# mikeoliphant/NeuralAudio

Measured on AMD Instinct MI355X. Metric: concurrent 48 kHz real-time streams + Msamples/s/GPU, NAM WaveNet Standard, higher is better.
Workload: dtype f32 (f16x3-split MFMA, f32 accumulate)

## Files before the change

include/neuralaudio_amd.h:

```cpp
#ifndef NEURALAUDIO_AMD_H
#define NEURALAUDIO_AMD_H

#include "NeuralAudioCApi.h"

#ifdef __cplusplus
extern "C" {
#endif

typedef struct NA_Batch NA_Batch;

NA_EXTERN const char* NA_GetLastError(void);
NA_EXTERN int NA_GetDeviceCount(void);
NA_EXTERN const char* NA_GetVersion(void);

NA_EXTERN NeuralModel* NA_CreateModelFromFileUtf8(NeuralModelLoader* loader, const char* utf8Path, int doPrewarm);
NA_EXTERN NeuralModel* NA_CreateModelFromString(NeuralModelLoader* loader, const char* jsonText, const char* extension, int doPrewarm);
NA_EXTERN void NA_SetDevice(NeuralModelLoader* loader, int device);
NA_EXTERN void NA_SetWaveNetMathMode(NeuralModelLoader* loader, int mathMode);
NA_EXTERN void NA_SetLSTMMathMode(NeuralModelLoader* loader, int mathMode);
NA_EXTERN void NA_SetCompositeModelLoadMode(NeuralModelLoader* loader, int loadMode);
NA_EXTERN int NA_IsQualityChangeRealtimeSafe(NeuralModel* model, float newQuality);
NA_EXTERN int NA_ProcessChecked(NeuralModel* model, float* input, float* output, size_t numSamples);
NA_EXTERN void NA_SetDefaultQualityScaleFactor(NeuralModelLoader* loader, float quality);
NA_EXTERN void NA_SetExternalSampleRate(NeuralModelLoader* loader, int sampleRate);
// ... 73 lines not shown
NA_EXTERN unsigned long long NA_ModelSnapshotFingerprint(NeuralModel* model);
NA_EXTERN int NA_BatchSaveStreams(NA_Batch* batch, const int* streams, int count, void* buf, size_t capacity, size_t* written);
NA_EXTERN int NA_BatchLoadStreams(NA_Batch* batch, const int* streams, int count, const void* buf, size_t bytes);
NA_EXTERN int NA_SaveModelState(NeuralModel* model, void* buf, size_t capacity, size_t* written);
NA_EXTERN int NA_LoadModelState(NeuralModel* model, const void* buf, size_t bytes);

typedef struct NA_MultiBatch NA_MultiBatch;
NA_EXTERN NA_MultiBatch* NA_MultiCreate(const int* devices, int numDevices);
NA_EXTERN void NA_MultiDestroy(NA_MultiBatch* multi);
NA_EXTERN int NA_MultiAddStreams(NA_MultiBatch* multi, NeuralModel* model, float quality, int count, int doPrewarm);
NA_EXTERN int NA_MultiCommit(NA_MultiBatch* multi);
NA_EXTERN int NA_MultiNumStreams(NA_MultiBatch* multi);
NA_EXTERN int NA_MultiNumShards(NA_MultiBatch* multi);
NA_EXTERN int NA_MultiShardRange(NA_MultiBatch* multi, int shard, int* begin, int* end, int* device);
NA_EXTERN int NA_MultiProcess(NA_MultiBatch* multi, const float* in, float* out, size_t n);
NA_EXTERN int NA_MultiSubmit(NA_MultiBatch* multi, const float* in, size_t n);
NA_EXTERN int NA_MultiCollect(NA_MultiBatch* multi, int ticket, float* out);
NA_EXTERN int NA_MultiSetQuality(NA_MultiBatch* multi, int stream, float quality);
NA_EXTERN int NA_MultiSetFanIn(NA_MultiBatch* multi, int mode);
NA_EXTERN const float* NA_MultiGatheredOutput(NA_MultiBatch* multi, int shard);
NA_EXTERN int NA_RcclAvailable(void);
NA_EXTERN int NA_ShardByCost(const double* cost, int n, int parts, int* bounds);
NA_EXTERN double NA_ModelStreamCost(NeuralModel* model, float quality);

NA_EXTERN int NA_ModelKernelInfo(NeuralModel* model, float quality, int streams, char* kernelBuf, int bufSize, float* inputLimit, int* rangeProven,
	int* weightsOk, int* packFactor);

NA_EXTERN float NA_BatchStreamInputLimit(NA_Batch* batch, int stream);
NA_EXTERN int NA_BatchStreamRangeEvents(NA_Batch* batch, int stream);

typedef struct NA_RenderJob
{
	NeuralModel* model;
	float quality;
	const float* input;
	float* output;
	size_t numSamples;
} NA_RenderJob;
typedef struct NA_RenderOptions
{
	size_t segmentSamples;
	size_t maxSamplesPerPass;
	double waitLimitMs;
} NA_RenderOptions;
typedef struct NA_RenderPlanInfo
{
	long long segments;
	int lead;
	long long segmentSamples;
	long long rowSamples;
	int passes;
	int streams;
	double estimatedMs;
	char kernel[64];
} NA_RenderPlanInfo;
NA_EXTERN int NA_RenderOffline(const NA_RenderJob* jobs, int numJobs, const NA_RenderOptions* opts);
NA_EXTERN int NA_RenderPlan(const NA_RenderJob* jobs, int numJobs, const NA_RenderOptions* opts, NA_RenderPlanInfo* info);

typedef struct NA_ResampleInfo {
	int externalRate, modelRate;
	int ticksExternal, ticksModel;
	int tapsUp, tapsDown;
	int quantum;
	int latencySamples;
	int prototypeLength;
} NA_ResampleInfo;
NA_EXTERN int NA_ResamplePlan(int externalRate, int modelRate, int quantum, NA_ResampleInfo* info);
NA_EXTERN int NA_ResamplePrototype(int externalRate, int modelRate, float* buf, int capacity);
NA_EXTERN long long NA_ResampleModelFrames(int externalRate, int modelRate, int quantum, long long externalSamples);
NA_EXTERN int NA_BatchSetResampling(NA_Batch* batch, int externalRate, int modelRate, int quantum, int maxFrames);
NA_EXTERN int NA_BatchGetResampleInfo(NA_Batch* batch, NA_ResampleInfo* info);
NA_EXTERN void NA_SetResampleToExternalRate(NeuralModelLoader* loader, int on);
NA_EXTERN int NA_GetProcessLatencySamples(NeuralModel* model);
NA_EXTERN int NA_GetModelProcessRate(NeuralModel* model);
NA_EXTERN int NA_RenderOfflineAtRate(const NA_RenderJob* jobs, int numJobs, const NA_RenderOptions* opts, int externalRate);
NA_EXTERN int NA_RenderPlanAtRate(const NA_RenderJob* jobs, int numJobs, const NA_RenderOptions* opts, int externalRate,
                                  NA_RenderPlanInfo* info, NA_ResampleInfo* resample);
NA_EXTERN int NA_MultiSetResampling(NA_MultiBatch* multi, int externalRate, int modelRate, int quantum, int maxFrames);
NA_EXTERN int NA_MultiGetResampleInfo(NA_MultiBatch* multi, NA_ResampleInfo* info);
#ifndef NA_RELEASE
NA_EXTERN int NA_DebugClassifyNam(const char* jsonText);
NA_EXTERN int NA_DebugPackedWeights(NeuralModel* model, int* packFactor, float* out, int capacity);
NA_EXTERN int NA_DebugSplitPlan(NeuralModel* model, int* stages, int stageCapacity, unsigned short* wsplit, long long wsplitCapacity, long long* wsplitCount);
NA_EXTERN void NA_DebugSetWaveNetSpec(int on);
NA_EXTERN int NA_DebugSetRecurrentQuadMin(int streams);
NA_EXTERN long long NA_DebugRecurrentQuadLaunches(void);
NA_EXTERN int NA_DebugRecurrentPlan(NeuralModel* model, int out[6]);
NA_EXTERN int NA_DebugRecurrentShapePlan(int cell, int hidden, int numLayers, int tailLayers, int tailWidth, int tailHistory, int rpl, int forceL2w, int out[6]);
NA_EXTERN int NA_DebugRecurrentKernel(int cell, int hidden, int numLayers, int tailLayers, int tailWidth, int tailHistory, int haveWT, int knobMask, int rpl,
	char* outName, int cap);
NA_EXTERN long long NA_DebugSnapshotLaunches(void);
NA_EXTERN void NA_DebugSetRcclApi(int mode, int failSendAt, int rendezvousMs);
NA_EXTERN int NA_DebugStallDevice(NA_Batch* batch, double milliseconds);
NA_EXTERN long long NA_DebugDeviceResourceCalls(void);
NA_EXTERN int NA_DebugResampleTap(NA_Batch* batch, float* modelIn, float* modelOut, long long capacityPerRow, int* frames);
NA_EXTERN void NA_DebugSetRenderTap(float* modelIn, float* modelOut, long long capacity);
NA_EXTERN void NA_DebugSetTraceBuffer(void* deviceBuffer);
NA_EXTERN int NA_DebugRunCabinetStage(NA_Batch* batch, float* hostRows, long stride, size_t n);
NA_EXTERN long long NA_DebugCabinetLaunches(void);
NA_EXTERN long long NA_DebugGateLaunches(void);
#endif

#ifdef __cplusplus
}
#endif
#endif
```

neuralaudio_amd/capi.py:

```python
import ctypes as C
import os

_HERE = os.path.dirname(os.path.abspath(__file__))
_SUFFIX = os.environ.get("NA_LIB_SUFFIX", "")
LIB_PATH = (os.path.join(os.path.dirname(_HERE), "tools", "variants", "libNeuralAudioCAPI%s.so" % _SUFFIX) if _SUFFIX
            else os.path.join(_HERE, "libNeuralAudioCAPI.so"))

LEGACY_SYMBOLS = [
    "CreateLoader", "DeleteLoader", "CreateModelFromFile", "DeleteModel", "SetLSTMLoadMode", "SetWaveNetLoadMode",
    "SetAudioInputLevelDBu", "SetDefaultMaxAudioBufferSize", "GetLoadMode", "IsStatic", "SetMaxAudioBufferSize",
    "GetRecommendedInputDBAdjustment", "GetRecommendedOutputDBAdjustment", "GetSampleRate", "Process",
]

NA_SYMBOLS = [
    "NA_GetLastError", "NA_GetDeviceCount", "NA_GetVersion", "NA_CreateModelFromFileUtf8", "NA_CreateModelFromString",
    "NA_SetDevice", "NA_SetDefaultQualityScaleFactor", "NA_SetExternalSampleRate", "NA_HasQualityScaling",
    "NA_GetQualityScaleFactor", "NA_SetQualityScaleFactor", "NA_GetReceptiveFieldSize", "NA_Prewarm", "NA_GetMetadata",
    "NA_GetModelVersion", "NA_BatchCreate", "NA_BatchDestroy", "NA_BatchAddStreams", "NA_BatchNumStreams",
    "NA_BatchSetQuality", "NA_BatchGetActiveSubModel", "NA_BatchPrewarm", "NA_BatchProcess", "NA_BatchProcessDevice",
    "NA_BatchSynchronize", "NA_BatchGetHipStream", "NA_BatchAlgorithmicBytesPerSample", "NA_BatchMacsPerSample",
    "NA_BatchStateBytes", "NA_BatchStreamPackFactor", "NA_BatchStreamKernelName", "NA_DebugSetTraceBuffer", "NA_DebugSetWaveNetSpec", "NA_DebugSetRecurrentQuadMin", "NA_DebugRecurrentQuadLaunches", "NA_RegisterHostBuffer", "NA_UnregisterHostBuffer", "NA_BatchStreamInputLimit", "NA_BatchRemoveStreams", "NA_MultiCreate", "NA_MultiDestroy", "NA_MultiAddStreams", "NA_MultiCommit", "NA_MultiNumStreams", "NA_MultiNumShards", "NA_MultiShardRange", "NA_MultiProcess", "NA_MultiSubmit", "NA_MultiCollect", "NA_MultiSetQuality", "NA_ShardByCost", "NA_ModelStreamCost", "NA_BatchNumLiveStreams", "NA_BatchIsLive", "NA_SetWaveNetMathMode", "NA_SetLSTMMathMode", "NA_SetCompositeModelLoadMode",
    "NA_IsQualityChangeRealtimeSafe", "NA_ProcessChecked", "NA_BatchSubmit", "NA_BatchCollect", "NA_BatchNextInput", "NA_BatchOutputView", "NA_BatchIsQualityChangeRealtimeSafe", "NA_DebugClassifyNam", "NA_DebugPackedWeights", "NA_DebugSplitPlan", "NA_ModelKernelInfo", "NA_BatchStreamRangeEvents", "NA_MultiSetFanIn", "NA_MultiGatheredOutput", "NA_RcclAvailable",
    "NA_BatchMarkTime", "NA_BatchWaitMarks", "NA_BatchElapsedMs", "NA_BatchUsesHalfLaunches", "NA_DebugSetRcclApi", "NA_BatchWaitOutputs", "NA_BatchUsesResidentLaunch", "NA_BatchSetResidentLaunch",
    "NA_BatchSetWaitLimitMs", "NA_BatchGetWaitLimitMs", "NA_BatchIsBroken", "NA_DebugStallDevice",
    "NA_RenderOffline", "NA_RenderPlan",
    "NA_BatchStreamSnapshotBytes", "NA_ModelSnapshotBytes", "NA_ModelSnapshotFingerprint", "NA_BatchSaveStreams", "NA_BatchLoadStreams",
    "NA_SaveModelState", "NA_LoadModelState", "NA_DebugSnapshotLaunches",
    "NA_ResamplePlan", "NA_ResamplePrototype", "NA_ResampleModelFrames", "NA_BatchSetResampling", "NA_BatchGetResampleInfo",
    "NA_SetResampleToExternalRate", "NA_GetProcessLatencySamples", "NA_GetModelProcessRate", "NA_DebugResampleTap",
    "NA_RenderOfflineAtRate", "NA_RenderPlanAtRate", "NA_DebugSetRenderTap", "NA_MultiSetResampling", "NA_MultiGetResampleInfo",
    "NA_BatchReserveStreams", "NA_BatchActivateStream", "NA_BatchParkStream", "NA_BatchIsParked", "NA_BatchFindParked", "NA_BatchNumParked",
    "NA_DebugDeviceResourceCalls", "NA_DebugRecurrentPlan", "NA_DebugRecurrentShapePlan", "NA_DebugRecurrentKernel",
    "NA_BatchEnableOutputStage", "NA_BatchSetStreamGain", "NA_BatchGetStreamGain", "NA_BatchHandover", "NA_BatchHandoverRemaining",
    "NA_BatchEnableCabinetStage", "NA_BatchGetCabinetInfo", "NA_BatchLoadIR", "NA_BatchUnloadIR", "NA_BatchSetStreamIR", "NA_BatchGetStreamIR",
    "NA_BatchStreamIRFadeRemaining", "NA_DebugRunCabinetStage", "NA_DebugCabinetLaunches",
    "NA_GateParamsFromDb", "NA_BatchEnableGateStage", "NA_BatchGetGateInfo", "NA_BatchSetStreamGate", "NA_BatchGetStreamGate",
    "NA_BatchStreamGateGain", "NA_DebugGateLaunches",
]


class NA_RenderJob(C.Structure):
    _fields_ = [("model", C.c_void_p), ("quality", C.c_float), ("input", C.POINTER(C.c_float)), ("output", C.POINTER(C.c_float)),
                ("numSamples", C.c_size_t)]


class NA_RenderOptions(C.Structure):
    _fields_ = [("segmentSamples", C.c_size_t), ("maxSamplesPerPass", C.c_size_t), ("waitLimitMs", C.c_double)]


class NA_RenderPlanInfo(C.Structure):
    _fields_ = [("segments", C.c_longlong), ("lead", C.c_int), ("segmentSamples", C.c_longlong), ("rowSamples", C.c_longlong),
                ("passes", C.c_int), ("streams", C.c_int), ("estimatedMs", C.c_double), ("kernel", C.c_char * 64)]


class NA_ResampleInfo(C.Structure):
    _fields_ = [("externalRate", C.c_int), ("modelRate", C.c_int), ("ticksExternal", C.c_int), ("ticksModel", C.c_int),
                ("tapsUp", C.c_int), ("tapsDown", C.c_int), ("quantum", C.c_int), ("latencySamples", C.c_int),
                ("prototypeLength", C.c_int)]


class NA_CabinetInfo(C.Structure):
    _fields_ = [("maxTaps", C.c_int), ("ringSamples", C.c_int), ("pieceSamples", C.c_int), ("numIRs", C.c_int), ("deviceBytes", C.c_longlong)]


class NA_GateParams(C.Structure):
    _fields_ = [("openPower", C.c_float), ("closePower", C.c_float), ("floorGain", C.c_float), ("detectorCoeff", C.c_float),
                ("attackSamples", C.c_int), ("holdSamples", C.c_int), ("releaseSamples", C.c_int)]


class NA_GateInfo(C.Structure):
    _fields_ = [("gainSamples", C.c_int), ("numGates", C.c_int), ("deviceBytes", C.c_longlong)]


_lib = None


def load_library():
    global _lib
    if _lib is not None:
        return _lib
    if not os.path.exists(LIB_PATH):
        raise OSError("libNeuralAudioCAPI.so not found at %s -- build it with `python -c 'import __graft_entry__ as g; "
                      "g.build()'` (there is no CPU fallback)" % LIB_PATH)
    lib = C.CDLL(LIB_PATH, mode=C.RTLD_GLOBAL)
    fp = C.POINTER(C.c_float)
    vp = C.c_void_p
    sig = {
        "CreateLoader": (vp, []),
        "DeleteLoader": (None, [vp]),
        "CreateModelFromFile": (vp, [vp, C.c_wchar_p]),
        "DeleteModel": (None, [vp]),
        "SetLSTMLoadMode": (None, [vp, C.c_int]),
        "SetWaveNetLoadMode": (None, [vp, C.c_int]),
        "SetAudioInputLevelDBu": (None, [vp, C.c_float]),
        "SetDefaultMaxAudioBufferSize": (None, [vp, C.c_int]),
        "GetLoadMode": (C.c_int, [vp]),
        "IsStatic": (C.c_bool, [vp]),
        "SetMaxAudioBufferSize": (None, [vp, C.c_int]),
        "GetRecommendedInputDBAdjustment": (C.c_float, [vp]),
        "GetRecommendedOutputDBAdjustment": (C.c_float, [vp]),
        "GetSampleRate": (C.c_float, [vp]),
        "Process": (None, [vp, fp, fp, C.c_size_t]),
        "NA_GetLastError": (C.c_char_p, []),
        "NA_GetDeviceCount": (C.c_int, []),
        "NA_GetVersion": (C.c_char_p, []),
# ... 54 lines not shown
        "NA_DebugDeviceResourceCalls": (C.c_longlong, []),
        "NA_BatchEnableOutputStage": (C.c_int, [vp]),
        "NA_BatchSetStreamGain": (C.c_int, [vp, C.c_int, C.c_float, C.c_int]),
        "NA_BatchGetStreamGain": (C.c_float, [vp, C.c_int]),
        "NA_BatchHandover": (C.c_int, [vp, C.c_int, C.c_int, C.c_float, C.c_int]),
        "NA_BatchHandoverRemaining": (C.c_int, [vp, C.c_int]),
        "NA_BatchEnableCabinetStage": (C.c_int, [vp, C.c_int]),
        "NA_BatchGetCabinetInfo": (C.c_int, [vp, C.POINTER(NA_CabinetInfo)]),
        "NA_BatchLoadIR": (C.c_int, [vp, fp, C.c_int]),
        "NA_BatchUnloadIR": (C.c_int, [vp, C.c_int]),
        "NA_BatchSetStreamIR": (C.c_int, [vp, C.c_int, C.c_int, C.c_int]),
        "NA_BatchGetStreamIR": (C.c_int, [vp, C.c_int]),
        "NA_BatchStreamIRFadeRemaining": (C.c_int, [vp, C.c_int]),
        "NA_DebugRunCabinetStage": (C.c_int, [vp, fp, C.c_long, C.c_size_t]),
        "NA_DebugCabinetLaunches": (C.c_longlong, []),
        "NA_GateParamsFromDb": (C.c_int, [C.c_int] + [C.c_float] * 7 + [C.POINTER(NA_GateParams)]),
        "NA_BatchEnableGateStage": (C.c_int, [vp]),
        "NA_BatchGetGateInfo": (C.c_int, [vp, C.POINTER(NA_GateInfo)]),
        "NA_BatchSetStreamGate": (C.c_int, [vp, C.c_int, C.POINTER(NA_GateParams), C.c_int]),
        "NA_BatchGetStreamGate": (C.c_int, [vp, C.c_int, C.POINTER(NA_GateParams)]),
        "NA_BatchStreamGateGain": (C.c_float, [vp, C.c_int]),
        "NA_DebugGateLaunches": (C.c_longlong, []),
        "NA_DebugRecurrentPlan": (C.c_int, [vp, C.POINTER(C.c_int)]),
        "NA_DebugRecurrentShapePlan": (C.c_int, [C.c_int] * 8 + [C.POINTER(C.c_int)]),
        "NA_DebugRecurrentKernel": (C.c_int, [C.c_int] * 9 + [C.c_char_p, C.c_int]),
        "NA_MultiCreate": (vp, [C.POINTER(C.c_int), C.c_int]),
        "NA_MultiDestroy": (None, [vp]),
        "NA_MultiAddStreams": (C.c_int, [vp, vp, C.c_float, C.c_int, C.c_int]),
        "NA_MultiCommit": (C.c_int, [vp]),
        "NA_MultiNumStreams": (C.c_int, [vp]),
        "NA_MultiNumShards": (C.c_int, [vp]),
        "NA_MultiShardRange": (C.c_int, [vp, C.c_int, C.POINTER(C.c_int), C.POINTER(C.c_int), C.POINTER(C.c_int)]),
        "NA_MultiProcess": (C.c_int, [vp, C.POINTER(C.c_float), C.POINTER(C.c_float), C.c_size_t]),
        "NA_MultiSubmit": (C.c_int, [vp, C.POINTER(C.c_float), C.c_size_t]),
        "NA_MultiCollect": (C.c_int, [vp, C.c_int, C.POINTER(C.c_float)]),
        "NA_MultiSetQuality": (C.c_int, [vp, C.c_int, C.c_float]),
        "NA_ShardByCost": (C.c_int, [C.POINTER(C.c_double), C.c_int, C.c_int, C.POINTER(C.c_int)]),
        "NA_ModelStreamCost": (C.c_double, [vp, C.c_float]),
        "NA_BatchStreamRangeEvents": (C.c_int, [vp, C.c_int]),
        "NA_MultiSetFanIn": (C.c_int, [vp, C.c_int]),
        "NA_MultiGatheredOutput": (vp, [vp, C.c_int]),
        "NA_RcclAvailable": (C.c_int, []),
        "NA_ModelKernelInfo": (C.c_int, [vp, C.c_float, C.c_int, C.c_char_p, C.c_int, fp, C.POINTER(C.c_int), C.POINTER(C.c_int), C.POINTER(C.c_int)]),
        "NA_BatchNumLiveStreams": (C.c_int, [vp]),
        "NA_BatchIsLive": (C.c_int, [vp, C.c_int]),
        "NA_SetWaveNetMathMode": (None, [vp, C.c_int]),
        "NA_SetLSTMMathMode": (None, [vp, C.c_int]),
        "NA_SetCompositeModelLoadMode": (None, [vp, C.c_int]),
        "NA_IsQualityChangeRealtimeSafe": (C.c_int, [vp, C.c_float]),
        "NA_ProcessChecked": (C.c_int, [vp, fp, fp, C.c_size_t]),
        "NA_BatchSubmit": (C.c_int, [vp, fp, C.c_size_t]),
        "NA_BatchCollect": (C.c_int, [vp, C.c_int, fp]),
        "NA_BatchNextInput": (fp, [vp, C.c_size_t]),
        "NA_BatchOutputView": (fp, [vp, C.c_int]),
        "NA_BatchIsQualityChangeRealtimeSafe": (C.c_int, [vp, C.c_int, C.c_float]),
        "NA_DebugClassifyNam": (C.c_int, [C.c_char_p]),
        "NA_DebugPackedWeights": (C.c_int, [vp, C.POINTER(C.c_int), C.POINTER(C.c_float), C.c_int]),
        "NA_RenderOffline": (C.c_int, [C.POINTER(NA_RenderJob), C.c_int, C.POINTER(NA_RenderOptions)]),
        "NA_RenderPlan": (C.c_int, [C.POINTER(NA_RenderJob), C.c_int, C.POINTER(NA_RenderOptions), C.POINTER(NA_RenderPlanInfo)]),
        "NA_BatchStreamSnapshotBytes": (C.c_longlong, [vp, C.c_int]),
        "NA_ModelSnapshotBytes": (C.c_longlong, [vp]),
        "NA_ModelSnapshotFingerprint": (C.c_ulonglong, [vp]),
        "NA_BatchSaveStreams": (C.c_int, [vp, C.POINTER(C.c_int), C.c_int, vp, C.c_size_t, C.POINTER(C.c_size_t)]),
        "NA_BatchLoadStreams": (C.c_int, [vp, C.POINTER(C.c_int), C.c_int, vp, C.c_size_t]),
        "NA_SaveModelState": (C.c_int, [vp, vp, C.c_size_t, C.POINTER(C.c_size_t)]),
        "NA_LoadModelState": (C.c_int, [vp, vp, C.c_size_t]),
        "NA_DebugSnapshotLaunches": (C.c_longlong, []),
        "NA_ResamplePlan": (C.c_int, [C.c_int, C.c_int, C.c_int, C.POINTER(NA_ResampleInfo)]),
        "NA_ResamplePrototype": (C.c_int, [C.c_int, C.c_int, fp, C.c_int]),
        "NA_ResampleModelFrames": (C.c_longlong, [C.c_int, C.c_int, C.c_int, C.c_longlong]),
        "NA_BatchSetResampling": (C.c_int, [vp, C.c_int, C.c_int, C.c_int, C.c_int]),
        "NA_BatchGetResampleInfo": (C.c_int, [vp, C.POINTER(NA_ResampleInfo)]),
        "NA_SetResampleToExternalRate": (None, [vp, C.c_int]),
        "NA_GetProcessLatencySamples": (C.c_int, [vp]),
        "NA_GetModelProcessRate": (C.c_int, [vp]),
        "NA_DebugResampleTap": (C.c_int, [vp, fp, fp, C.c_longlong, C.POINTER(C.c_int)]),
        "NA_RenderOfflineAtRate": (C.c_int, [C.POINTER(NA_RenderJob), C.c_int, C.POINTER(NA_RenderOptions), C.c_int]),
        "NA_RenderPlanAtRate": (C.c_int, [C.POINTER(NA_RenderJob), C.c_int, C.POINTER(NA_RenderOptions), C.c_int, C.POINTER(NA_RenderPlanInfo),
                                          C.POINTER(NA_ResampleInfo)]),
        "NA_DebugSetRenderTap": (None, [fp, fp, C.c_longlong]),
        "NA_MultiSetResampling": (C.c_int, [vp, C.c_int, C.c_int, C.c_int, C.c_int]),
        "NA_MultiGetResampleInfo": (C.c_int, [vp, C.POINTER(NA_ResampleInfo)]),
        "NA_DebugSplitPlan": (C.c_int, [vp, C.POINTER(C.c_int), C.c_int, C.POINTER(C.c_ushort), C.c_longlong, C.POINTER(C.c_longlong)]),
    }
    for name, (res, args) in sig.items():
        try:
            fn = getattr(lib, name)
        except AttributeError:
            if os.environ.get("NA_LIB_SUFFIX") and name.startswith("NA_"):
                continue
            raise
        fn.restype = res
        fn.argtypes = args
    _lib = lib
    return lib


def last_error():
    return load_library().NA_GetLastError().decode("utf-8", "replace")


def device_count():
    return int(load_library().NA_GetDeviceCount())
```

neuralaudio_amd/csrc/capi.cpp:

```cpp
#include <cstring>
#include <cwchar>
#include <string>

#include "neuralaudio_amd.h"
#include "multi_gpu.h"
#include "offline_render.h"
#include "resample.h"
#include "stream_snapshot.h"
#include "neural_model_impl.h"
#include "lstm_launch.h"
#include "wavenet_launch.h"
#include "wavenet_plan.h"
#include "tuning.h"

struct NeuralModel
{
	NeuralAudio::NeuralModel* model;
};

struct NeuralModelLoader
{
	NeuralAudio::NeuralModelLoader* loader;
};

// ... 198 lines not shown
}

int NA_ProcessChecked(NeuralModel* model, float* input, float* output, size_t numSamples)
{
	if (!model || !output)
	{
		SetError("Process: null argument");
		return -1;
	}
	const int rc = Guard([&] { model->model->Process(input, output, numSamples); });
	if (rc != 0) memset(output, 0, numSamples * sizeof(float));
	return rc;
}

void NA_SetWaveNetMathMode(NeuralModelLoader* loader, int mathMode)
{
	if (loader) loader->loader->SetWaveNetMathMode(mathMode == 1 ? NeuralAudio::EMathMode::StdMath : NeuralAudio::EMathMode::FastMath);
}

void NA_SetLSTMMathMode(NeuralModelLoader* loader, int mathMode)
{
	if (loader) loader->loader->SetLSTMMathMode(mathMode == 1 ? NeuralAudio::EMathMode::StdMath : NeuralAudio::EMathMode::FastMath);
}

void NA_SetCompositeModelLoadMode(NeuralModelLoader* loader, int loadMode)
{
	if (loader) loader->loader->SetCompositeModelLoadMode(loadMode == 1 ? NeuralAudio::ECompositeModelLoadMode::OnDemand : NeuralAudio::ECompositeModelLoadMode::LoadAll);
}

int NA_IsQualityChangeRealtimeSafe(NeuralModel* model, float newQuality)
{
	return (model && model->model->IsQualityChangeRealtimeSafe(newQuality)) ? 1 : 0;
}

#ifndef NA_RELEASE
int NA_DebugClassifyNam(const char* jsonText)
{
	int r = -1;
	Guard([&] {
		const na::Json j = na::Json::Parse(jsonText ? jsonText : "");
		const std::string v = (j.IsObject() && j.Contains("version") && j.At("version").IsString()) ? j.At("version").AsString() : "";
		r = (na::NAMIsA2(v) ? 1 : 0) | (na::NAMIsA2Standard(j) ? 2 : 0);
	});
	return r;
}
#endif

#ifndef NA_RELEASE
int NA_DebugPackedWeights(NeuralModel* model, int* packFactor, float* out, int capacity)
{
	int r = -1;
	Guard([&] {
		NeuralAudio::GpuModel* gm = model ? dynamic_cast<NeuralAudio::GpuModel*>(model->model) : nullptr;
		if (!gm) throw std::runtime_error("NA_DebugPackedWeights: not a model of this library");
		const auto& lm = gm->GetLoadedModel();
		if (lm->subModels.size() != 1 || lm->subModels[0].desc->kind != na::MODEL_WAVENET)
		{
			if (packFactor) *packFactor = 1;
			r = 0;
			return;
		}
		const na::WaveNetDesc& wn = lm->subModels[0].desc->wavenet;
		const int P = na::WaveNetPackFactor(wn);
		if (packFactor) *packFactor = P;
		if (P < 2)
		{
			r = 0;
			return;
		}
		const bool dense = na::Tuning::Get().wnDense != 0 && na::WaveNetPackCanBeDense(wn, P);
		const na::WaveNetDesc v = na::PackWaveNetDesc(wn, P, dense);
		na::ValidateWaveNetDesc(v);
		const na::WaveNetPlan plan = na::BuildPackedWaveNetPlan(wn, P, dense);
		if (plan.pack != P || plan.splitFastT != 2) throw std::runtime_error("NA_DebugPackedWeights: the packed plan is not a fast split-kernel plan");
		r = (int)v.weights.size();
		if (out)
			for (int i = 0; i < r && i < capacity; i++) out[i] = v.weights[(size_t)i];
	});
	return r;
}
#endif

#ifndef NA_RELEASE
int NA_DebugSplitPlan(NeuralModel* model, int* stages, int stageCapacity, unsigned short* wsplit, long long wsplitCapacity, long long* wsplitCount)
{
	int r = -1;
	Guard([&] {
		NeuralAudio::GpuModel* gm = model ? dynamic_cast<NeuralAudio::GpuModel*>(model->model) : nullptr;
		if (!gm) throw std::runtime_error("NA_DebugSplitPlan: not a model of this library");
		const auto& lm = gm->GetLoadedModel();
		if (lm->subModels.size() != 1 || lm->subModels[0].desc->kind != na::MODEL_WAVENET) throw std::runtime_error("NA_DebugSplitPlan: not a WaveNet");
		const na::WaveNetPlan plan = na::BuildWaveNetPlan(lm->subModels[0].desc->wavenet, true);
		static_assert(sizeof(na::WnSplitStage) == 16 * sizeof(int), "16 ints per stage");
		r = (int)plan.sstages.size();
		if (stages) memcpy(stages, plan.sstages.data(), sizeof(na::WnSplitStage) * (size_t)std::min(r, stageCapacity));
		if (wsplitCount) *wsplitCount = (long long)plan.wsplit.size();
		if (wsplit) memcpy(wsplit, plan.wsplit.data(), sizeof(uint16_t) * (size_t)std::min<long long>((long long)plan.wsplit.size(), wsplitCapacity));
	});
	return r;
}
#endif

#ifndef NA_RELEASE
int NA_DebugRecurrentShapePlan(int cell, int hidden, int numLayers, int tailLayers, int tailWidth, int tailHistory, int rpl, int forceL2w, int out[6])
{
	if (!out || (cell != 0 && cell != 1) || hidden < 1 || numLayers < 0 || tailLayers < 0) return -1;
	const na::RecurrentPlan p = na::RecurrentWavePlan(cell == 1 ? na::LSTM_CELL_GRU : na::LSTM_CELL_LSTM, hidden, numLayers, tailLayers, tailWidth, tailHistory, true, rpl, forceL2w);
	out[0] = p.runs; out[1] = p.waves; out[2] = p.rowsPerLane; out[3] = p.l2w; out[4] = p.headInLoop; out[5] = (int)p.ldsBytes;
	return na::RecurrentWaveShape(hidden, numLayers, tailLayers > 0 ? tailWidth : 0, tailLayers > 0 ? tailHistory : 0) ? 1 : 0;
}
#endif

#ifndef NA_RELEASE
int NA_DebugRecurrentKernel(int cell, int hidden, int numLayers, int tailLayers, int tailWidth, int tailHistory, int haveWT, int knobMask, int rpl, char* outName, int cap)
{
	if ((cell != 0 && cell != 1) || hidden < 1 || numLayers < 0 || tailLayers < 0 || knobMask < -1 || knobMask > 63) return -1;
	const int b = knobMask;
	const na::RecurrentKnobs k = b < 0 ? na::RecurrentKnobs::FromTuning()
		: na::RecurrentKnobs{ (b & 1) != 0, (b & 2) != 0, (b & 4) != 0, (b & 8) != 0, (b & 16) != 0, rpl > 0 ? rpl : 1, (b & 32) != 0 };
	const na::RecurrentKernel kernel = na::RecurrentKernelFor(cell == 1 ? na::LSTM_CELL_GRU : na::LSTM_CELL_LSTM, hidden, numLayers, tailLayers, tailWidth, tailHistory,
		haveWT != 0, k).kernel;
	if (outName && cap > 0) snprintf(outName, (size_t)cap, "%s", na::RecurrentKernelName(kernel));
	return (int)kernel;
}
#endif

#ifndef NA_RELEASE
int NA_DebugRecurrentPlan(NeuralModel* model, int out[6])
{
	int r = -1;
	Guard([&] {
		NeuralAudio::GpuModel* gm = model ? dynamic_cast<NeuralAudio::GpuModel*>(model->model) : nullptr;
		if (!gm || !out) throw std::runtime_error("NA_DebugRecurrentPlan: not a model of this library");
		const auto& lm = gm->GetLoadedModel();
		if (lm->subModels.size() != 1 || lm->subModels[0].desc->kind != na::MODEL_LSTM) throw std::runtime_error("NA_DebugRecurrentPlan: not a recurrent model");
		const na::LSTMDesc& d = lm->subModels[0].desc->lstm;
		int tailWidth = 0, tailHistory = 0;
		na::RecurrentTailDims(d, tailWidth, tailHistory);
		const na::RecurrentPlan p = na::RecurrentWavePlan(d.cell == na::CELL_GRU ? na::LSTM_CELL_GRU : na::LSTM_CELL_LSTM, d.hiddenSize, d.numLayers, (int)d.tail.size(),
			tailWidth, tailHistory);
		out[0] = p.runs; out[1] = p.waves; out[2] = p.rowsPerLane; out[3] = p.l2w; out[4] = p.headInLoop; out[5] = (int)p.ldsBytes;
		r = 0;
	});
	return r;
}
#endif

void NA_SetDevice(NeuralModelLoader* loader, int device)
{
	if (loader) loader->loader->SetDevice(device);
}

void NA_SetDefaultQualityScaleFactor(NeuralModelLoader* loader, float quality)
{
	if (loader) loader->loader->SetDefaultQualityScaleFactor(quality);
}

void NA_SetExternalSampleRate(NeuralModelLoader* loader, int sampleRate)
{
	if (loader) loader->loader->SetExternalSampleRate(sampleRate);
}

int NA_HasQualityScaling(NeuralModel* model) { return (model && model->model->HasQualityScaling()) ? 1 : 0; }

float NA_GetQualityScaleFactor(NeuralModel* model) { return model ? model->model->GetQualityScaleFactor() : 1.0f; }

void NA_SetQualityScaleFactor(NeuralModel* model, float quality)
{
	if (model) Guard([&] { model->model->SetQualityScaleFactor(quality); });
}

int NA_GetReceptiveFieldSize(NeuralModel* model) { return model ? model->model->GetReceptiveFieldSize() : -1; }

int NA_Prewarm(NeuralModel* model)
{
	if (!model) return -1;
	return Guard([&] { model->model->Prewarm(); });
}

int NA_GetMetadata(NeuralModel* model, const char* fieldName, char* buf, int bufSize)
// ... 962 lines not shown
```

neuralaudio_amd/csrc/tuning.cpp:

```cpp
#include "tuning.h"

#include <cstdlib>
#include <cstring>

namespace na
{
	namespace
	{
#ifndef NA_NO_TUNING
		bool Has(const char* name) { return getenv(name) != nullptr; }
		int Int(const char* name, int dflt)
		{
			const char* e = getenv(name);
			return e ? atoi(e) : dflt;
		}
		bool IsZero(const char* name)
		{
			const char* e = getenv(name);
			return e != nullptr && atoi(e) == 0;
		}
#endif
		Tuning Parse()
		{
			Tuning t;
#ifndef NA_NO_TUNING
			if (const char* e = getenv("NA_WN_KERNEL")) t.wnKernel = !strcmp(e, "split") ? 1 : (!strcmp(e, "frame") ? 2 : (!strcmp(e, "generic") ? 3 : 0));
			t.wnPack = Int("NA_WN_PACK", -1);
			t.wnPadOff = IsZero("NA_WN_PAD");
			t.wnNtOff = IsZero("NA_WN_NT");
			t.wnNtFromMB = Int("NA_WN_NT_MB", 400);
			t.wnDense = Int("NA_WN_DENSE", -1);
			t.spT = Int("NA_SP_T", 0);
			t.spSpb = Int("NA_SP_SPB", 0);
			t.spGen = Has("NA_SP_GEN");
			t.wnSpecOff = IsZero("NA_WN_SPEC") || Has("NA_SP_T") || Has("NA_SP_GEN");
			t.spNoT1 = Has("NA_SP_NO_T1");
			t.spReverse = Has("NA_SP_REVERSE");
			t.frPrefetch = Int("NA_FR_PF", 1);
			t.frSpb = Int("NA_FR_SPB", 0);
			t.traceBlock = Int("NA_TRACE_BLOCK", 0);
			t.traceChain = Int("NA_TRACE_CHAIN", 0);
			t.lstmNoDpp = Has("NA_LSTM_NO_DPP");
			t.gruNoDpp = Has("NA_GRU_NO_DPP");
			t.lstmLaneKernel = Has("NA_LSTM_LANE_KERNEL");
			t.lstmNoWaveRt = Has("NA_LSTM_NO_WAVE_RT");
			t.recL2w = Int("NA_REC_L2W", 0) != 0;
			t.recQuadMin = Int("NA_REC_QUAD_MIN", -1);
			t.recNoDpp32 = Has("NA_REC_NO_DPP32");
			t.recNoSkew = Has("NA_REC_NOSKEW");
			t.recNoPipe = Has("NA_REC_NOPIPE");
			t.recPipeMax = Int("NA_REC_PIPE_MAX", 0);
			t.recRpl = Int("NA_REC_RPL", 1);
			t.hostChains = Int("NA_HOST_CHAINS", 2);
			t.hostHalvesOff = IsZero("NA_HOST_HALVES");
			t.hostDirect = !IsZero("NA_HOST_DIRECT");
			t.batchSerial = Has("NA_BATCH_SERIAL");
			t.batchNoGraph = Has("NA_BATCH_NO_GRAPH");
			t.residentOn = Int("NA_RESIDENT", 0) != 0;
			t.residentHostRing = Int("NA_RESIDENT_HOST_RING", 0) != 0;
			t.residentDelayUs = Int("NA_RESIDENT_DELAY_US", 0);
			t.residentGrid = Int("NA_RESIDENT_GRID", 0);
			t.residentIdleUs = Int("NA_RESIDENT_IDLE_US", 200);
#endif
			return t;
		}
	}

	const Tuning& Tuning::Get()
	{
		static const Tuning t = Parse();
		return t;
	}
}
```

neuralaudio_amd/csrc/tuning.h:

```cpp
#pragma once

namespace na
{
	struct Tuning
	{
		int wnKernel = 0;
		int wnPack = -1;
		int wnDense = -1;
		int wnNtFromMB = 400;
		bool wnNtOff = false;
		bool wnPadOff = false;
		bool wnSpecOff = false;
		int spT = 0;
		int spSpb = 0;
		bool spGen = false;
		bool spNoT1 = false;
		bool spReverse = false;
		int frPrefetch = 1;
		int frSpb = 0;
		int traceBlock = 0;
		int traceChain = 0;
		bool lstmNoDpp = false;
		bool gruNoDpp = false;
		bool lstmLaneKernel = false;
		bool lstmNoWaveRt = false;
		bool recL2w = false;
		int recQuadMin = -1;
		bool recNoDpp32 = false;
		bool recNoSkew = false;
		bool recNoPipe = false;
		int recPipeMax = 0;
		int recRpl = 1;
		int hostChains = 2;
		bool hostHalvesOff = false;
		bool hostDirect = true;
		bool batchSerial = false;
		bool batchNoGraph = false;
		bool residentOn = false;
		bool residentHostRing = false;
		int residentDelayUs = 0;
		int residentGrid = 0;
		int residentIdleUs = 200;

		static const Tuning& Get();
	};
}
```

neuralaudio_amd/csrc/wavenet_dev.h:

```cpp
#pragma once

#include <cstdint>

namespace na
{
	constexpr int WN_TILE = 16;
	constexpr int WN_MAX_TILES = 8;
	constexpr int WN_MAX_FRAMES = WN_TILE * WN_MAX_TILES;
	constexpr int WN_MAX_RINGS = 64;
	constexpr int WN_HEADER_F4 = WN_MAX_RINGS / 4;
	constexpr int WN_RANGE_EVENT_SLOT = WN_MAX_RINGS - 1;

	constexpr int WN_COMPACT_MAX_HISTORY = 32;
	constexpr int WnRingKeep(int ringFrames) { return ringFrames < WN_MAX_FRAMES ? ringFrames / 3 : ringFrames - WN_MAX_FRAMES; }
	constexpr bool WnCompactSafeFrames(int n) { return (n >= 1 && n <= 32) || n == 64 || n == 128; }

	enum WnStageType : int
	{
		WN_ST_RECHANNEL_COND = 0,
		WN_ST_LAYER = 1,
		WN_ST_ARRAY_LINK = 2,
		WN_ST_HEAD_DENSE_OUT = 3,
		WN_ST_HEAD_CONV_OUT = 4,
	};

	enum WnStageFlags : int
	{
		WN_FLAG_LEAKY = 1,
		WN_FLAG_NEED_OUTPUT = 2,
		WN_FLAG_PUBLISH = 4,
		WN_FLAG_BIAS = 8,
		WN_FLAG_STD_TANH = 16,
		WN_FLAG_FOLD = 32,
	};

	struct WnStage
	{
		int type;
		int flags;
		int G;
		int ksize;
		int dilation;
		int ring_id;
		int ring_off;
		int ring_frames;
		int out_ring_id;
		int out_ring_off;
		int out_ring_frames;
		int out_G;
		int a4_off;
		int a4_floats;
		int vec_off;
		int pk_conv_off;
		int pk_w1_off;
		int reserved[15];
	};
	static_assert(sizeof(WnStage) == 128, "stage descriptors are 128-byte records");


	struct WnSplitStage
	{
		int type;
		int flags;
		int G;
		int Gp;
		int ksize;
		int dilation;
		int ring_off;
		int ring_frames;
		int ring_id;
		int out_ring_off;
		int out_ring_frames;
		int out_ring_id;
		int out_G;
		int a_off;
		int a_ops;
		int reserved;
	};
	static_assert(sizeof(WnSplitStage) == 64, "split stage descriptors are 64-byte records");

	constexpr int WN_GENERIC_MAX_CHANNELS = 128;
	constexpr int WN_COL_STRIDE = 128;

	struct WnPrewarmLayer
	{
		int kind;
		int cin, cout, ksize;
		int act;
		int wconv;
		int bconv;
		int wmix;
		int w1, b1;
		int ring_id;
		int need_output;
		int last_of_array;
		int rechannel;
		int rech_in;
		int dilation;
	};

	struct WnModelDev
	{
		const WnStage* stages;
		const float* wpack;
		const float* wpk;
		const int* ring_frames;
		int nstages;
		int wpack_f4;
		int max_a4_floats;
		int max_ksize;
		int wpk_floats;
		int nrings;
		int state_f4;
		float head_scale;
		const WnSplitStage* sstages;
		const void* wsplit;
		int wsplit_quads;
		int max_split_ops;
		int max_G;
		int split_fast_T;
		int spec_arch;
		float cond_limit;
		int compact_rings;
		int saturate;
	};

	enum WnSpecArch : int
	{
		WN_SPEC_NONE = 0,
		WN_SPEC_STD = 1,
		WN_SPEC_LITE = 2,
		WN_SPEC_LITE16 = 3,
		WN_SPEC_A2FULL = 4,
		WN_SPEC_A2LITE = 5,
	};
}
```

neuralaudio_amd/csrc/wavenet_launch.h:

```cpp
#pragma once

#include <cstring>
#include <vector>

#include <hip/hip_runtime_api.h>

#include "device_resources.h"
#include "tuning.h"
#include "wavenet_dev.h"

namespace na
{
	constexpr int WN_FRAME_MAX_GROUPS = 8;
	struct WnFrameGroup
	{
		const WnModelDev* model;
		float* state;
		const int* slots;
		const int* rows;
		int numStreams, slot0, row0;
		int pack;
	};
	hipError_t LaunchWaveNetFrameFused(const WnFrameGroup* groups, int numGroups, const float* in, float* out, long inStride, long outStride, int n,
		hipStream_t stream);
// ... 31 lines not shown
			entries.clear();
		}
		void NewGeneration(unsigned long g)
		{
			if (g != generation) Clear();
			generation = g;
		}
		hipError_t Ensure(const void* fresh, size_t bytes, hipStream_t stream, const void** dev)
		{
			for (const Entry& e : entries)
				if (e.host.size() == bytes && memcmp(e.host.data(), fresh, bytes) == 0)
				{
					*dev = e.dev;
					return hipSuccess;
				}
			hipStreamCaptureStatus capturing = hipStreamCaptureStatusNone;
			(void)hipStreamIsCapturing(stream, &capturing);
			if (capturing != hipStreamCaptureStatusNone) return hipErrorStreamCaptureUnsupported;
			if (entries.size() >= 16) Clear();
			Entry e;
			hipError_t err = CountedHipMalloc(&e.dev, bytes);
			if (err != hipSuccess) return err;
			err = hipMemcpy(e.dev, fresh, bytes, hipMemcpyHostToDevice);
			if (err != hipSuccess)
			{
				(void)CountedHipFree(e.dev);
				return err;
			}
			e.host.assign(static_cast<const char*>(fresh), static_cast<const char*>(fresh) + bytes);
			*dev = e.dev;
			entries.push_back(std::move(e));
			return hipSuccess;
		}
	};
	hipError_t LaunchWaveNetSpecTable(const WnFrameGroup* groups, int numGroups, const float* in, float* out, long inStride, long outStride, int n,
		hipStream_t stream, WnLaunchTable& table);

	constexpr int RESIDENT_RING = 64;
	struct ResidentCmd
	{
		const float* in;
		float* out;
		long inStride, outStride;
		unsigned long long seq;
		unsigned long long check;
		unsigned long long pad[2];
	};
#ifdef __HIPCC__
	__host__ __device__
#endif
	inline unsigned long long ResidentCmdCheck(unsigned long long in, unsigned long long out, unsigned long long inStride, unsigned long long outStride, unsigned long long seq)
	{
		return seq * 0x9E3779B97F4A7C15ull + in * 0xC2B2AE3D27D4EB4Full + out * 0x165667B19E3779F9ull + inStride * 0xD6E8FEB86659FD93ull + outStride * 0xFF51AFD7ED558CCDull + 1ull;
	}
	struct ResidentCtrl
	{
		unsigned long long exitAfter;
		unsigned long long pad0[7];
		ResidentCmd cmd[RESIDENT_RING];
	};
	struct ResidentStatus
	{
		unsigned long long completed;
		unsigned long long pad1[7];
	};
	static_assert(sizeof(ResidentCmd) == 64 && sizeof(ResidentCtrl) == 64 + 64 * RESIDENT_RING && sizeof(ResidentStatus) == 64, "command ring layout");
	struct ResidentArgs
	{
		const ResidentCtrl* ctrl;
		ResidentStatus* status;
		unsigned* doneCount;
		unsigned* wgDone;
		unsigned long long base;
		int numBlocks;
		unsigned idleTicks;
		unsigned startDelay;
	};
	hipError_t LaunchWaveNetSpecResident(const WnFrameGroup* groups, int numGroups, int n, const ResidentArgs& ra, hipStream_t stream, int* gridOut);
	int WaveNetSpecResidentGrid(const WnFrameGroup* groups, int numGroups, int n);

	bool WaveNetSpecEnabled();
	void SetWaveNetSpecEnabled(bool on);
	int WaveNetSpecArchId(const WnSplitStage* stages, int nstages, int stateF4, int wsplitQuads);

	hipError_t LaunchWaveNetGeneric(const WnPrewarmLayer* layers, int numLayers, const float* weights, const int* ringOffF4, const int* ringFrames,
		const int* ringG, int nrings, int stateF4, int maxChannels, float headScale, float condLimit, bool saturate, float* state, const int* slots, const int* rows,
		int numStreams, int slot0, int row0, const float* in, float* out, long inStride, long outStride, int n, hipStream_t stream);

	hipError_t LaunchWaveNetFrame(const WnModelDev& m, float* state, const int* slots, const int* rows, int numStreams, const float* in,
		float* out, long inStride, long outStride, int n, hipStream_t stream, int slot0 = 0, int row0 = 0);

	void SetWaveNetTraceBuffer(long long* deviceBuffer);
	long long* GetWaveNetTraceBuffer();

	hipError_t LaunchWaveNetPrewarmColumns(const WnPrewarmLayer* layers, int numLayers, const float* weights, float* cols,
		hipStream_t stream);

	hipError_t LaunchWaveNetFillRings(float* state, int stateF4, const int* slots, int numStreams, int numRings, const int* ringOffF4,
		const int* ringFrames, const int* ringG, const float* cols, hipStream_t stream, bool splitFormat, const int* sub = nullptr, int pack = 1,
		bool zero = false);

	hipError_t LaunchWaveNetRearm(float* state, int stateF4, const int* entries, int numEntries, int numRings, const int* ringOffF4,
		const int* ringFrames, const int* ringG, const float* cols, hipStream_t stream, bool splitFormat, int pack);
}
```

neuralaudio_amd/csrc/wavenet_plan.cpp:

```cpp
#include "wavenet_plan.h"
#include "frame_lds.h"

#include <algorithm>
#include <cmath>
#include <cstring>
#include <functional>
#include <sstream>
#include <stdexcept>

namespace na
{
	static int CeilDiv(int a, int b) { return (a + b - 1) / b; }

	size_t WaveNetDesc::ExpectedNumWeights() const
	{
		size_t n = 0;
		for (const auto& a : arrays)
		{
			const size_t c = (size_t)a.channels;
			n += c * a.inputSize;
			for (size_t l = 0; l < a.kernelSizes.size(); l++)
			{
				n += c * c * a.kernelSizes[l] + c;
				n += c * a.conditionSize;
// ... 19 lines not shown
	{
		if (desc.arrays.empty()) throw std::runtime_error("WaveNet without layer arrays");
		const int numArrays = (int)desc.arrays.size();
		int rings = 0;
		for (int a = 0; a < numArrays; a++)
		{
			const WnArrayCfg& cfg = desc.arrays[a];
			if (cfg.channels < 1 || cfg.headSize < 1 || cfg.inputSize < 1) throw std::runtime_error("WaveNet layer array with a zero-sized dimension");
			if (cfg.channels > WN_GENERIC_MAX_CHANNELS || cfg.headSize > WN_GENERIC_MAX_CHANNELS || cfg.inputSize > WN_GENERIC_MAX_CHANNELS)
				throw std::runtime_error("WaveNet channels > 128 are not supported");
			if (cfg.headKernelSize > 1 && (cfg.channels > 64 || cfg.headSize > 64))
				throw std::runtime_error("WaveNet: a conv head on a layer array wider than 64 channels is not supported");
			if (cfg.conditionSize != 1) throw std::runtime_error("WaveNet condition_size != 1 is not supported");
			if (cfg.kernelSizes.size() != cfg.dilations.size() || cfg.kernelSizes.empty())
				throw std::runtime_error("WaveNet kernel_sizes/dilations mismatch");
			for (size_t l = 0; l < cfg.kernelSizes.size(); l++)
				if (cfg.kernelSizes[l] < 1 || cfg.dilations[l] < 1) throw std::runtime_error("WaveNet kernel_size / dilation must be >= 1");
			if (cfg.headKernelSize < 1 || cfg.headDilation < 1) throw std::runtime_error("WaveNet head kernel_size / dilation must be >= 1");
			rings += (int)cfg.kernelSizes.size() + (cfg.headKernelSize > 1 ? 1 : 0);
			if (a > 0)
			{
				if (desc.arrays[a - 1].headSize != cfg.channels || cfg.inputSize != desc.arrays[a - 1].channels)
					throw std::runtime_error("WaveNet layer arrays do not chain (head_size/input_size mismatch)");
				if (desc.arrays[a - 1].headKernelSize != 1)
					throw std::runtime_error("WaveNet: head kernel > 1 is only supported on the last layer array");
			}
		}
		if (desc.arrays[0].inputSize != 1) throw std::runtime_error("WaveNet first layer array must have input_size 1");
		if (rings > WN_MAX_RINGS) throw std::runtime_error("WaveNet has more than 64 conv layers (unsupported)");
		const size_t expected = desc.ExpectedNumWeights();
		if (expected != desc.weights.size())
		{
			std::stringstream str;
			str << "Wrong number of weights. Expected " << expected << " but got " << desc.weights.size();
			throw std::runtime_error(str.str());
		}
	}


	static uint16_t FloatToHalfBits(float f)
	{
		uint32_t x;
		memcpy(&x, &f, 4);
		const uint32_t sign = (x >> 16) & 0x8000u;
		x &= 0x7fffffffu;
		if (x >= 0x7f800000u) return (uint16_t)(sign | 0x7c00u | (x > 0x7f800000u ? 0x200u : 0u));
		if (x >= 0x477ff000u) return (uint16_t)(sign | 0x7c00u);
		if (x < 0x33000001u) return (uint16_t)sign;
		int e = (int)(x >> 23) - 127;
		uint32_t m = (x & 0x7fffffu) | 0x800000u;
		int shift = (e < -14) ? (13 + (-14 - e)) : 13;
		uint32_t half = m >> shift;
		const uint32_t rem = m & ((1u << shift) - 1u), halfway = 1u << (shift - 1);
		if (rem > halfway || (rem == halfway && (half & 1u))) half++;
		if (e < -14) return (uint16_t)(sign | half);
		half += (uint32_t)(e + 15 - 1) << 10;
		return (uint16_t)(sign | half);
	}

	static float HalfBitsToFloat(uint16_t h)
	{
		const uint32_t sign = (uint32_t)(h & 0x8000u) << 16;
		const int e = (h >> 10) & 0x1f;
		const uint32_t m = h & 0x3ffu;
		float v;
		if (e == 0) v = std::ldexp((float)m, -24);
		else if (e == 31) v = m ? NAN : INFINITY;
		else v = std::ldexp((float)(m | 0x400u), e - 25);
		return sign ? -v : v;
	}

	static int LaneMode(int channels) { return channels <= 4 ? 1 : (channels <= 8 ? 2 : 4); }

	namespace
	{
		struct Builder
		{
			const WaveNetDesc& desc;
			WaveNetPlan plan;
			size_t cursor = 0;

			int pack = 1;
			bool foldOk = false;
			bool exactRings = false;
			bool compactOk = false;

			explicit Builder(const WaveNetDesc& d, int packStreams = 1, bool exact = false) : desc(d), pack(packStreams), exactRings(exact) {}

			int Take(size_t n)
			{
				const size_t off = cursor;
				cursor += n;
				return (int)off;
			}

			float W(int off) const { return desc.weights[(size_t)off]; }

			int AllocF4(int nF4)
			{
				const int off = (int)(plan.wpack.size() / 4);
				plan.wpack.resize(plan.wpack.size() + (size_t)nF4 * 4, 0.0f);
				return off;
			}

			int AddRing(int channels, int history, int dilation, bool firstOfArray = true)
			{
				WnRingInfo r;
				r.channels = channels;
				r.G = CeilDiv(channels, 4);
			const bool exact = exactRings && !firstOfArray && dilation >= WN_MAX_FRAMES && history >= 2 * WN_MAX_FRAMES && history % WN_TILE == 0;
				const int H = CeilDiv(history, WN_TILE) * WN_TILE;
				const bool compact = compactOk && history > 0 && H <= WN_COMPACT_MAX_HISTORY;
				if (compact) plan.compactRings = true;
				r.frames = exact ? history : (compact ? 3 * H : H + WN_MAX_FRAMES);
				r.offF4 = plan.stateF4;
				plan.stateF4 += (r.frames / WN_TILE) * r.G * WN_TILE;
				plan.rings.push_back(r);
				if ((int)plan.rings.size() > WN_MAX_RINGS) throw std::runtime_error("WaveNet has more than 64 conv layers (unsupported)");
				return (int)plan.rings.size() - 1;
			}

			int AllocPk(int nFloats)
			{
				const int off = (int)plan.wpk.size();
				plan.wpk.resize(plan.wpk.size() + (size_t)((nFloats + 15) & ~15), 0.0f);
				return off;
			}

			int PackConvPk(int wOff, int cin, int cout, int ksize, int CPin, int CPout)
			{
				const int off = AllocPk(ksize * CPin * CPout);
				for (int k = 0; k < ksize; k++)
					for (int c = 0; c < cin; c++)
						for (int o = 0; o < cout; o++) plan.wpk[(size_t)off + ((size_t)k * CPin + c) * CPout + o] = W(wOff + (o * cin + c) * ksize + k);
				return off;
			}

			int PackDensePk(int wOff, int cin, int cout, int CPin, int CPout)
			{
				const int off = AllocPk(CPin * CPout);
				for (int c = 0; c < cin; c++)
					for (int o = 0; o < cout; o++) plan.wpk[(size_t)off + (size_t)c * CPout + o] = W(wOff + o * cin + c);
				return off;
			}

			int PackConvA4(int wOff, int cin, int cout, int ksize, int G)
			{
				const int off = AllocPk(ksize * 64 * G);
				for (int k = 0; k < ksize; k++)
					for (int lane = 0; lane < 64; lane++)
						for (int og = 0; og < G; og++)
						{
							const int o = 4 * og + (lane & 3), c = lane >> 2;
							if (o < cout && c < cin) plan.wpk[(size_t)off + ((size_t)k * 64 + lane) * G + og] = W(wOff + (o * cin + c) * ksize + k);
						}
				return off;
			}

			int PackDenseA4(int wOff, int cin, int cout, int G)
			{
				const int off = AllocPk(64 * G);
				for (int lane = 0; lane < 64; lane++)
					for (int og = 0; og < G; og++)
					{
						const int o = 4 * og + (lane & 3), c = lane >> 2;
						if (o < cout && c < cin) plan.wpk[(size_t)off + (size_t)lane * G + og] = W(wOff + o * cin + c);
// ... 130 lines not shown
					for (int c = 0; c < C * cfg.headKernelSize; c++) row += std::fabs((double)W(wh + o * C * cfg.headKernelSize + c));
					rowMax = std::max(rowMax, row);
					if (bh >= 0) bMax = std::max(bMax, std::fabs((double)W(bh + o)));
				}
				rangeHeadGain *= rowMax;
				rangeHeadAdd = rangeHeadAdd * rowMax + bMax;
				RangeNote(rangeHeadGain, rangeHeadAdd);
			}

			void FinishRange()
			{
				double limit = 32752.0;
				for (const auto& c : rangeCons)
				{
					const double room = 32752.0 - c.second;
					limit = std::min(limit, room <= 0.0 ? 0.0 : (c.first > 0.0 ? room / c.first : 32752.0));
				}
				plan.splitRangeProven = limit >= kSplitMinInputLimit;
				plan.condLimit = (float)(plan.splitRangeProven ? limit : std::min(32752.0, 32752.0 / std::max(1e-6, linearGainMax)));
				plan.splitWeightsOk = weightAbsMax <= 32752.0 && (matrixPeakMin >= 1.0 / 4096.0 || matrixPeakMin == 1e300);
			}

			int NewSplitOps(int count)
			{
				const int first = (int)(plan.wsplit.size() / 512);
				plan.wsplit.resize(plan.wsplit.size() + (size_t)count * 512, 0);
				return first;
			}

			void FillSplitBlock(int opHi, int opLo, int rowBase, int kbBase, int cout, int cin, const std::function<float(int, int)>& w, int loSlot = 0)
			{
				for (int o = 0; o < cout; o++)
					for (int c = 0; c < cin; c++)
					{
						const int row = rowBase + o, q = kbBase + c / 4, r = c % 4;
						if (row > 15 || q > 3) throw std::runtime_error("internal: split operand block out of range");
						const float v = w(o, c);
						const uint16_t hi = FloatToHalfBits(v);
						const uint16_t lo = FloatToHalfBits(v - HalfBitsToFloat(hi));
						const size_t lane = (size_t)q * 16 + row;
						plan.wsplit[(size_t)opHi * 512 + lane * 8 + r] = hi;
						plan.wsplit[(size_t)opHi * 512 + lane * 8 + 4 + r] = hi;
						plan.wsplit[(size_t)opLo * 512 + lane * 8 + loSlot + r] = lo;
					}
			}

			void FillSplitMerged(int opHi, int Gp, int cout, int cin, const std::function<float(int, int)>& w, int opLo = -1, int loSlot = 0)
			{
				for (int p = 0; p < 4 / Gp; p++) FillSplitBlock(opHi, opLo < 0 ? opHi + 1 : opLo, 4 * Gp * p, Gp * p, cout, cin, w, loSlot);
			}

			void FillSplitAux(int op, int Gp, int cout, int condOff, int oneOff, int cpad = 1 << 20)
			{
				for (int p = 0; p < 4 / Gp; p++)
					for (int o = 0; o < cout; o++)
					{
						const float wc = condOff >= 0 ? W(condOff + o) : 0.0f, w1 = oneOff >= 0 ? W(oneOff + o) : 0.0f;
						const uint16_t wch = FloatToHalfBits(wc), wcl = FloatToHalfBits(wc - HalfBitsToFloat(wch));
						const uint16_t w1h = FloatToHalfBits(w1), w1l = FloatToHalfBits(w1 - HalfBitsToFloat(w1h));
						const bool halfGroups = cpad == 2;
						const size_t kblock = (size_t)Gp * p + (halfGroups ? (size_t)(o / 4) : (size_t)((o / cpad) * (cpad / 4)));
						const size_t lane = kblock * 16 + (size_t)(4 * Gp * p + o);
						uint16_t* e = &plan.wsplit[(size_t)op * 512 + lane * 8];
						if (halfGroups && ((o / 2) & 1)) { e[1] = w1h; e[3] = w1l; e[5] = wch; e[6] = wch; e[7] = wcl; }
						else { e[0] = wch; e[1] = w1h; e[2] = wch; e[3] = w1l; e[4] = wcl; }
					}
			}

			void FillSplitFoldAux(int op, int Gp, int cout, int condOff, int oneOff)
			{
				if (Gp < 2) throw std::runtime_error("internal: folded aux operand needs two k-blocks per tile slot");
				for (int p = 0; p < 4 / Gp; p++)
					for (int o = 0; o < cout; o++)
					{
						const float wc = condOff >= 0 ? W(condOff + o) : 0.0f, w1 = oneOff >= 0 ? W(oneOff + o) : 0.0f;
						const uint16_t wch = FloatToHalfBits(wc), wcl = FloatToHalfBits(wc - HalfBitsToFloat(wch));
						const uint16_t w1h = FloatToHalfBits(w1), w1l = FloatToHalfBits(w1 - HalfBitsToFloat(w1h));
						const size_t row = (size_t)(4 * Gp * p + o), kb = (size_t)(Gp * p);
						uint16_t* e = &plan.wsplit[(size_t)op * 512 + (kb * 16 + row) * 8];
						uint16_t* e2 = &plan.wsplit[(size_t)op * 512 + ((kb + 1) * 16 + row) * 8];
						e[4] = wch; e[5] = w1h; e[6] = wch; e[7] = w1l;
						e2[4] = wcl;
					}
			}

			static WnSplitStage EmptySplit(int type)
			{
				WnSplitStage st = {};
				st.type = type;
				st.ring_off = -1; st.ring_id = -1;
				st.out_ring_off = -1; st.out_ring_id = -1;
				return st;
			}

			void SplitRing(WnSplitStage& st, int ringId)
			{
				st.ring_id = ringId;
				st.ring_off = plan.rings[ringId].offF4;
				st.ring_frames = plan.rings[ringId].frames;
			}

			void SplitOutRing(WnSplitStage& st, int ringId)
			{
				st.out_ring_id = ringId;
				st.out_ring_off = plan.rings[ringId].offF4;
				st.out_ring_frames = plan.rings[ringId].frames;
				st.out_G = plan.rings[ringId].G;
			}

			void BuildSplit(const std::vector<std::vector<int>>& layerRing, const std::vector<int>& headRing)
			{
				cursor = 0;
				const int numArrays = (int)desc.arrays.size();
				int prevHeadW = -1, prevHeadB = -1;
				for (int a = 0; a < numArrays; a++)
				{
					const WnArrayCfg& cfg = desc.arrays[a];
					const int C = cfg.channels, G = CeilDiv(C, 4), Gp = LaneMode(C);
					const int numLayers = (int)cfg.kernelSizes.size();
					const bool lastArray = (a == numArrays - 1);
					plan.maxG = std::max(plan.maxG, G);
					const int cpad = pack > 1 ? C / pack : (1 << 20);
					const int groupsPerStream = pack > 1 ? cpad / 4 : 4;
					const int rechOff = Take((size_t)C * cfg.inputSize);
					RangeRechannel(a, cfg, rechOff);
					if (a == 0)
					{
						WnSplitStage st = EmptySplit(WN_ST_RECHANNEL_COND);
						st.G = G; st.Gp = Gp;
						st.a_ops = 1;
						st.a_off = NewSplitOps(st.a_ops) * 64;
						FillSplitAux(st.a_off / 64, Gp, C, rechOff, -1, cpad);
						st.reserved = groupsPerStream;
						SplitOutRing(st, layerRing[a][0]);
						st.flags = WN_FLAG_PUBLISH;
						plan.sstages.push_back(st);
					}
					else
					{
						const WnArrayCfg& prev = desc.arrays[a - 1];
						const int GpO = LaneMode(prev.channels), Po = 4 / GpO, Pn = 4 / Gp, NC = std::max(Po, Pn);
						WnSplitStage st = EmptySplit(WN_ST_ARRAY_LINK);
						st.G = CeilDiv(prev.channels, 4); st.Gp = GpO; st.ksize = Gp;
						st.a_ops = 4 * NC + 1;
						st.a_off = NewSplitOps(st.a_ops) * 64;
						const int op0 = st.a_off / 64;
						for (int u = 0; u < NC; u++)
						{
							const int pn = u % Pn, po = u % Po;
							FillSplitBlock(op0 + 4 * u, op0 + 4 * u + 1, 4 * Gp * pn, GpO * po, prev.headSize, prev.channels,
								[&](int o, int c) { return W(prevHeadW + o * prev.channels + c); });
							FillSplitBlock(op0 + 4 * u + 2, op0 + 4 * u + 3, 4 * Gp * pn, GpO * po, C, cfg.inputSize,
								[&](int o, int c) { return W(rechOff + o * cfg.inputSize + c); });
						}
						if (prev.hasHeadBias)
						{
							st.flags |= WN_FLAG_BIAS;
							FillSplitAux(op0 + 4 * NC, Gp, prev.headSize, -1, prevHeadB);
						}
						SplitOutRing(st, layerRing[a][0]);
						st.flags |= WN_FLAG_PUBLISH;
						plan.sstages.push_back(st);
					}

					for (int l = 0; l < numLayers; l++)
					{
						const int K = cfg.kernelSizes[l];
						const int wconv = Take((size_t)C * C * K);
						const int bconv = Take((size_t)C);
						const int wmix = Take((size_t)C * cfg.conditionSize);
						const int w1 = Take((size_t)C * C);
						const int b1 = Take((size_t)C);
						const bool lastLayer = (l == numLayers - 1);
						const bool needOutput = !(lastLayer && lastArray);
						RangeLayer(a == 0 && l == 0, cfg, K, wconv, bconv, wmix, w1, b1, needOutput);

						WnSplitStage st = EmptySplit(WN_ST_LAYER);
						st.G = G; st.Gp = Gp; st.ksize = K; st.dilation = cfg.dilations[l];
						st.a_ops = 2 * K + 4;
						st.a_off = NewSplitOps(st.a_ops) * 64;
						const int op0 = st.a_off / 64;
						const bool fold = foldOk && pack == 1 && K == 3 && Gp >= 2 && cfg.conditionSize == 1;
						for (int k = 0; k < K; k++)
							FillSplitMerged(op0 + 2 * k, Gp, C, C, [&](int o, int c) { return W(wconv + (o * C + c) * K + k); },
								(fold && k == 1) ? op0 + 1 : -1, (fold && k == 1) ? 4 : 0);
						if (fold) FillSplitFoldAux(op0 + 2 * K - 1, Gp, C, wmix, bconv);
						else FillSplitAux(op0 + 2 * K, Gp, C, wmix, bconv, cpad);
						st.reserved = groupsPerStream;
						FillSplitMerged(op0 + 2 * K + 1, Gp, C, C, [&](int o, int c) { return W(w1 + o * C + c); });
						if (fold)
						{
							FillSplitFoldAux(op0 + 2 * K + 2, Gp, C, -1, b1);
							st.flags |= WN_FLAG_FOLD;
						}
						else FillSplitAux(op0 + 2 * K + 3, Gp, C, -1, b1);
						if (needOutput) st.flags |= WN_FLAG_NEED_OUTPUT;
						SplitRing(st, layerRing[a][l]);
						if (cfg.activation == ACT_LEAKYRELU) st.flags |= WN_FLAG_LEAKY;
						else if (desc.mathMode == MATH_STD) st.flags |= WN_FLAG_STD_TANH;
						if (!lastLayer)
						{
							st.flags |= WN_FLAG_PUBLISH;
							SplitOutRing(st, layerRing[a][l + 1]);
						}
						plan.sstages.push_back(st);
					}

					const int wh = Take((size_t)cfg.headSize * C * cfg.headKernelSize);
					const int bh = cfg.hasHeadBias ? Take((size_t)cfg.headSize) : -1;
					RangeHead(cfg, wh, bh, lastArray);
					if (lastArray)
					{
						const int Kh = cfg.headKernelSize;
						WnSplitStage st = EmptySplit(Kh == 1 ? WN_ST_HEAD_DENSE_OUT : WN_ST_HEAD_CONV_OUT);
						st.G = G; st.Gp = Gp; st.ksize = Kh; st.dilation = cfg.headDilation;
						st.a_ops = 2 * Kh + 1;
						st.a_off = NewSplitOps(st.a_ops) * 64;
						const int op0 = st.a_off / 64;
						for (int k = 0; k < Kh; k++)
							FillSplitMerged(op0 + 2 * k, Gp, pack > 1 ? cfg.headSize : 1, C, [&](int o, int c) { return W(wh + (o * C + c) * Kh + k); });
						if (cfg.hasHeadBias)
						{
							st.flags |= WN_FLAG_BIAS;
							FillSplitAux(op0 + 2 * Kh, Gp, pack > 1 ? cfg.headSize : 1, -1, bh);
						}
						if (Kh > 1)
						{
							SplitRing(st, headRing[a]);
							SplitOutRing(st, headRing[a]);
						}
						plan.sstages.push_back(st);
					}
					else
					{
						prevHeadW = wh;
						prevHeadB = bh;
					}
				}
				for (const WnSplitStage& st : plan.sstages) plan.maxSplitOps = std::max(plan.maxSplitOps, st.a_ops);
				FinishRange();
				plan.splitFastT = 2;
				for (const WnSplitStage& st : plan.sstages)
				{
					if (st.a_ops > 16 || st.G != st.Gp || st.type == WN_ST_HEAD_CONV_OUT || (st.type == WN_ST_LAYER && st.ksize != 3)) plan.splitFastT = 0;
					if (plan.splitFastT && (st.Gp == 1 || (st.type == WN_ST_ARRAY_LINK && st.ksize == 1))) plan.splitFastT = 4;
				}
			}

			void BuildGenericOnly()
			{
				const int numArrays = (int)desc.arrays.size();
				cursor = 0;
				for (int a = 0; a < numArrays; a++)
				{
					const WnArrayCfg& cfg = desc.arrays[a];
					const int C = cfg.channels;
					const int numLayers = (int)cfg.kernelSizes.size();
					const int rechOff = Take((size_t)C * cfg.inputSize);
					RangeRechannel(a, cfg, rechOff);
					for (int l = 0; l < numLayers; l++)
					{
						const int K = cfg.kernelSizes[l];
						WnPrewarmLayer pw = {};
						pw.kind = 0;
						pw.cin = C; pw.cout = C; pw.ksize = K;
						pw.act = (cfg.activation == ACT_LEAKYRELU) ? 1 : (desc.mathMode == MATH_STD ? 2 : 0);
						pw.wconv = Take((size_t)C * C * K);
						pw.bconv = Take((size_t)C);
						pw.wmix = Take((size_t)C * cfg.conditionSize);
						pw.w1 = Take((size_t)C * C);
						pw.b1 = Take((size_t)C);
						pw.ring_id = AddRing(C, (K - 1) * cfg.dilations[l], cfg.dilations[l], l == 0);
						pw.need_output = 1;
						pw.last_of_array = (l == numLayers - 1) ? 1 : 0;
						pw.rechannel = (l == 0) ? rechOff : -1;
						pw.rech_in = cfg.inputSize;
						pw.dilation = cfg.dilations[l];
						plan.prewarm.push_back(pw);
						RangeLayer(a == 0 && l == 0, cfg, K, pw.wconv, pw.bconv, pw.wmix, pw.w1, pw.b1, !(l == numLayers - 1 && a == numArrays - 1));
					}
					WnPrewarmLayer pw = {};
					pw.kind = 1;
					pw.cin = C; pw.cout = cfg.headSize; pw.ksize = cfg.headKernelSize;
					pw.wconv = Take((size_t)cfg.headSize * C * cfg.headKernelSize);
					pw.bconv = cfg.hasHeadBias ? Take((size_t)cfg.headSize) : -1;
					pw.wmix = -1; pw.w1 = -1; pw.b1 = -1;
					pw.ring_id = (cfg.headKernelSize > 1) ? AddRing(C, (cfg.headKernelSize - 1) * cfg.headDilation, cfg.headDilation) : -1;
					pw.rechannel = -1;
					pw.dilation = cfg.headDilation;
					plan.prewarm.push_back(pw);
					RangeHead(cfg, pw.wconv, pw.bconv, a == numArrays - 1);
				}
				plan.headScale = W(Take(1));
				plan.stateF4 = CeilDiv(plan.stateF4, 16) * 16;
				FinishRange();
			}

			void Build()
			{
				ValidateWaveNetDesc(desc);

				plan.arrays = desc.arrays;
				plan.receptiveField = desc.ReceptiveFieldSize();
				compactOk = exactRings;
				for (const WnArrayCfg& cfg : desc.arrays)
				{
					if (cfg.headKernelSize != 1) compactOk = false;
					for (int k : cfg.kernelSizes)
						if (k > 3) compactOk = false;
				}
				plan.stateF4 = WN_HEADER_F4;
				plan.genericOk = true;
				for (const WnArrayCfg& cfg : desc.arrays)
				{
					plan.maxChannels = std::max(plan.maxChannels, std::max(cfg.channels, std::max(cfg.headSize, cfg.inputSize)));
					(void)cfg;
				}
				if (plan.maxChannels > 16)
				{
					plan.genericOnly = true;
					BuildGenericOnly();
// ... 87 lines not shown
						else if (desc.mathMode == MATH_STD) st.flags |= WN_FLAG_STD_TANH;
						if (!(lastLayer && lastArray)) st.flags |= WN_FLAG_NEED_OUTPUT;
						if (!lastLayer)
						{
							st.flags |= WN_FLAG_PUBLISH;
							SetOutRing(st, layerRing[a][l + 1]);
						}
						plan.stages.push_back(st);

						WnPrewarmLayer pw = {};
						pw.kind = 0;
						pw.cin = C; pw.cout = C; pw.ksize = K;
						pw.act = (cfg.activation == ACT_LEAKYRELU) ? 1 : (desc.mathMode == MATH_STD ? 2 : 0);
						pw.wconv = wconv; pw.bconv = bconv; pw.wmix = wmix; pw.w1 = w1; pw.b1 = b1;
						pw.ring_id = layerRing[a][l];
						pw.need_output = 1;
						pw.last_of_array = lastLayer ? 1 : 0;
						pw.rechannel = (l == 0) ? rechOff : -1;
						pw.rech_in = cfg.inputSize;
						pw.dilation = d;
						plan.prewarm.push_back(pw);
					}

					const int wh = Take((size_t)cfg.headSize * C * cfg.headKernelSize);
					const int bh = cfg.hasHeadBias ? Take((size_t)cfg.headSize) : -1;

					WnPrewarmLayer pw = {};
					pw.kind = 1;
					pw.cin = C; pw.cout = cfg.headSize; pw.ksize = cfg.headKernelSize;
					pw.wconv = wh; pw.bconv = bh; pw.wmix = -1; pw.w1 = -1; pw.b1 = -1;
					pw.ring_id = headRing[a];
					pw.rechannel = -1;
					pw.dilation = cfg.headDilation;
					plan.prewarm.push_back(pw);

					if (lastArray)
					{
						if (cfg.headKernelSize == 1)
						{
							WnStage st = EmptyStage(WN_ST_HEAD_DENSE_OUT);
							st.vec_off = AllocF4(16);
							st.G = CeilDiv(C, 4);
							st.pk_w1_off = PackDensePk(wh, C, 1, 16, 1);
							if (cfg.hasHeadBias)
							{
								st.flags |= WN_FLAG_BIAS;
								SetVec(st, 0, bh, cfg.headSize);
							}
							plan.stages.push_back(st);
						}
						else
						{
							WnStage st = EmptyStage(WN_ST_HEAD_CONV_OUT);
							st.G = CeilDiv(C, 4);
							st.vec_off = AllocF4(16);
							st.ksize = cfg.headKernelSize;
							st.dilation = cfg.headDilation;
							st.pk_conv_off = PackConvPk(wh, C, 1, cfg.headKernelSize, 4 * st.G, 1);
							if (cfg.hasHeadBias)
							{
								st.flags |= WN_FLAG_BIAS;
								SetVec(st, 0, bh, cfg.headSize);
							}
							SetRing(st, headRing[a]);
							SetOutRing(st, headRing[a]);
							plan.stages.push_back(st);
						}
					}
					else
					{
						prevHeadW = wh;
						prevHeadB = bh;
					}
				}

				plan.headScale = W(Take(1));
				BuildSplit(layerRing, headRing);
				for (const WnStage& st : plan.stages) plan.maxA4Floats = std::max(plan.maxA4Floats, st.a4_floats);
				plan.stateF4 = CeilDiv(plan.stateF4, 16) * 16;
			}
		};
	}

	WaveNetPlan BuildWaveNetPlan(const WaveNetDesc& desc, bool splitStateFormat)
	{
		Builder b(desc, 1, splitStateFormat);
		b.foldOk = true;
		b.Build();
		return std::move(b.plan);
	}

	void CheckWaveNetRunnable(const WaveNetDesc& desc)
	{
		const WaveNetPlan plan = BuildWaveNetPlan(desc);
		if (!plan.genericOnly)
		{
			for (size_t a = 0; a < desc.arrays.size(); a++)
			{
				const WnArrayCfg& cfg = desc.arrays[a];
				const int G = (cfg.channels + 3) / 4;
				for (size_t l = 0; l < cfg.kernelSizes.size(); l++)
				{
					const int K = cfg.kernelSizes[l];
					if (FrameModelFits(FrameLayerBlockFloats(K, G))) continue;
					std::stringstream str;
					str << "WaveNet layer array " << a << ", layer " << l << ": kernel size " << K << " at " << cfg.channels
					    << " channels needs " << FrameLaunchLdsBytes(FrameLayerBlockFloats(K, G), 2, 1, 1) << " bytes of LDS on the f32 frame kernel (limit "
					    << FRAME_LDS_LIMIT << "); the largest kernel size at this width is " << FrameMaxKernelSize(G);
					throw std::runtime_error(str.str());
				}
			}
			if (!FrameModelFits(plan.maxA4Floats))
			{
				std::stringstream str;
				str << "WaveNet: the largest staged weight block (" << plan.maxA4Floats << " floats) needs " << FrameLaunchLdsBytes(plan.maxA4Floats, 2, 1, 1)
				    << " bytes of LDS on the f32 frame kernel (limit " << FRAME_LDS_LIMIT << ")";
				throw std::runtime_error(str.str());
			}
			return;
		}
		const std::string who = "WaveNet with layer arrays wider than 16 channels (f16-split arithmetic only): ";
		if (!plan.splitWeightsOk)
			throw std::runtime_error(who + "the weights do not fit the (hi, lo) f16 operand format (a weight beyond 32752, or a weight matrix whose largest entry is below 2^-12)");
		bool allLeaky = true;
		for (const WnArrayCfg& cfg : desc.arrays) allLeaky = allLeaky && cfg.activation == ACT_LEAKYRELU;
		if ((!plan.splitRangeProven && !allLeaky) || plan.condLimit < kSplitMinInputLimit)
		{
			std::stringstream str;
			str << who << "the static range bound leaves no input limit of at least " << kSplitMinInputLimit
			    << " (the layers can drive the residual stream or the head accumulator beyond the f16 range)";
			throw std::runtime_error(str.str());
		}
	}

	int WaveNetPackFactor(const WaveNetDesc& desc)
	{
		int maxPad = 0;
		for (const WnArrayCfg& cfg : desc.arrays)
		{
			maxPad = std::max(maxPad, CeilDiv(cfg.channels, 4) * 4);
			if (cfg.headKernelSize != 1 || cfg.conditionSize != 1) return 1;
			for (int k : cfg.kernelSizes)
				if (k != 3) return 1;
		}
		if (desc.arrays.back().headSize != 1) return 1;
		return maxPad <= 4 ? 4 : (maxPad <= 8 ? 2 : 1);
	}

	bool WaveNetPackCanBeDense(const WaveNetDesc& desc, int P)
	{
		return P == 4 && desc.arrays.size() == 2 && desc.arrays[0].channels == 4 && desc.arrays[1].channels == 2;
	}

	WaveNetDesc PackWaveNetDesc(const WaveNetDesc& desc, int P, bool dense)
	{
		WaveNetDesc v;
		v.mathMode = desc.mathMode;
		const int numArrays = (int)desc.arrays.size();
		if (dense && !WaveNetPackCanBeDense(desc, P)) throw std::runtime_error("internal: this WaveNet has no dense pack");
		std::vector<int> cpad((size_t)numArrays);
		for (int a = 0; a < numArrays; a++)
			cpad[(size_t)a] = (dense && a == numArrays - 1) ? desc.arrays[(size_t)a].channels
				: (P > 1 ? CeilDiv(desc.arrays[(size_t)a].channels, 4) * 4 : 4 * LaneMode(desc.arrays[(size_t)a].channels));
		size_t pos = 0;
		auto take = [&](size_t n) { const size_t at = pos; pos += n; return at; };
		for (int a = 0; a < numArrays; a++)
		{
			const WnArrayCfg& cfg = desc.arrays[(size_t)a];
			const bool last = (a == numArrays - 1);
			const int C = cfg.channels, Cp = cpad[(size_t)a], Cv = P * Cp;
// ... 134 lines not shown
```

neuralaudio_amd/csrc/wavenet_plan.h:

```cpp
#pragma once

#include <cstdint>
#include <vector>

#include "model_desc.h"
#include "wavenet_dev.h"

namespace na
{
	struct WnRingInfo
	{
		int G;
		int frames;
		int offF4;
		int channels;
	};

	constexpr double kSplitMinInputLimit = 8.0;

	struct WaveNetPlan
	{
		std::vector<WnStage> stages;
		std::vector<float> wpack;
		std::vector<float> wpk;
		std::vector<WnRingInfo> rings;
		std::vector<WnPrewarmLayer> prewarm;
		std::vector<WnSplitStage> sstages;
		std::vector<uint16_t> wsplit;
		int maxSplitOps = 0;
		int maxG = 1;
		int splitFastT = 0;
		int maxChannels = 0;
		int pack = 1;
		bool packDense = false;
		bool isVirtual() const { return !packedWeights.empty(); }
		std::vector<float> packedWeights;
		bool genericOnly = false;
		bool genericOk = false;
		int stateF4 = 0;
		int maxA4Floats = 0;
		float headScale = 0.0f;
		float condLimit = 32752.0f;
		bool compactRings = false;
		bool splitRangeProven = true;
		bool splitWeightsOk = true;
		int receptiveField = 0;

		double AlgorithmicBytesPerSample(int blockFrames) const;
		double MacsPerSample() const;

		std::vector<WnArrayCfg> arrays;
	};

	WaveNetPlan BuildWaveNetPlan(const WaveNetDesc& desc, bool splitStateFormat = false);
	void CheckWaveNetRunnable(const WaveNetDesc& desc);
	int WaveNetPackFactor(const WaveNetDesc& desc);
	bool WaveNetWantsPadding(const WaveNetDesc& desc);
	bool WaveNetPackCanBeDense(const WaveNetDesc& desc, int P);
	WaveNetDesc PackWaveNetDesc(const WaveNetDesc& desc, int P, bool dense = false);
	WaveNetPlan BuildPackedWaveNetPlan(const WaveNetDesc& desc, int P, bool dense = false);
}
```

neuralaudio_amd/csrc/wavenet_spec_impl.h:

```cpp
#pragma once

#include <algorithm>
#include <atomic>
#include <cstddef>
#include <cstdlib>

#include <hip/hip_runtime.h>

#include "device_once.h"
#include <cstring>
#include <type_traits>
#include <vector>

#include "tuning.h"
#include "wavenet_split_dev.h"

namespace na
{
	namespace spk
	{
		using namespace sp;

#ifndef NA_SPK_NT_DIL
#define NA_SPK_NT_DIL 256
#endif
#ifndef NA_SPK_NT_LD
#define NA_SPK_NT_LD 0
#endif
#ifndef NA_SPK_NT_ST
#define NA_SPK_NT_ST 0
#endif
#ifndef NA_SPK_DELAY
#define NA_SPK_DELAY 0
#endif
#ifndef NA_SPK_AUX2
#define NA_SPK_AUX2 0
#endif
		typedef __attribute__((address_space(3))) char* LdsPtr;
		__device__ __forceinline__ u32x4 LdsRead16(unsigned addr) { return *reinterpret_cast<__attribute__((address_space(3))) const u32x4*>((LdsPtr)(size_t)addr); }
		__device__ __forceinline__ u32x2 LdsRead8(unsigned addr) { return *reinterpret_cast<__attribute__((address_space(3))) const u32x2*>((LdsPtr)(size_t)addr); }
		__device__ __forceinline__ void LdsWrite16(unsigned addr, u32x4 v) { *reinterpret_cast<__attribute__((address_space(3))) u32x4*>((LdsPtr)(size_t)addr) = v; }

		template <bool COH>
		__device__ __forceinline__ float LoadIn(const float* p)
		{
			if constexpr (COH) return __builtin_bit_cast(float, __hip_atomic_load(reinterpret_cast<const unsigned*>(p), __ATOMIC_RELAXED, __HIP_MEMORY_SCOPE_SYSTEM));
			else return *p;
		}
		template <bool COH>
		__device__ __forceinline__ void StoreOut(float* p, float v)
		{
			if constexpr (COH) __hip_atomic_store(reinterpret_cast<unsigned*>(p), __builtin_bit_cast(unsigned, v), __ATOMIC_RELAXED, __HIP_MEMORY_SCOPE_SYSTEM);
			else *p = v;
		}

		struct ArchA1Base
		{
			static constexpr int K(int, int) { return 3; }
			static constexpr int HEADK = 1;
			static constexpr bool LEAKY = false;
			static constexpr int T = 2, CHUNK = 10;
			static constexpr bool COARSE = false;
			static constexpr bool GUARDHIST = false;
			static constexpr bool FOLD = false;
			static constexpr int SKEW = 0;
			static constexpr bool COMPACT = true;
#ifndef NA_A1_NT_DIL
#define NA_A1_NT_DIL 128
#endif
			static constexpr int NT_DIL = NA_A1_NT_DIL;
		};
#ifndef NA_SPK_SKEW
#define NA_SPK_SKEW 0
#endif
		struct ArchStd : ArchA1Base
		{
			static constexpr int SKEW = NA_SPK_SKEW;
			static constexpr bool FOLD = true;
			static constexpr int NA = 2;
			static constexpr int CH[2] = { 16, 8 };
			static constexpr int NLA[2] = { 10, 10 };
			static constexpr int DIL[2][16] = { { 1, 2, 4, 8, 16, 32, 64, 128, 256, 512 }, { 1, 2, 4, 8, 16, 32, 64, 128, 256, 512 } };
		};
		struct ArchLite : ArchA1Base
		{
			static constexpr int NA = 2;
			static constexpr int CH[2] = { 16, 8 };
			static constexpr int NLA[2] = { 7, 13 };
			static constexpr int DIL[2][16] = { { 1, 2, 4, 8, 16, 32, 64 }, { 128, 256, 512, 1, 2, 4, 8, 16, 32, 64, 128, 256, 512 } };
		};
		struct ArchLite16 : ArchA1Base
		{
			static constexpr int NA = 2;
			static constexpr int CH[2] = { 16, 16 };
			static constexpr int NLA[2] = { 7, 13 };
			static constexpr int DIL[2][16] = { { 1, 2, 4, 8, 16, 32, 64 }, { 128, 256, 512, 1, 2, 4, 8, 16, 32, 64, 128, 256, 512 } };
		};

		struct ArchLite16T1 : ArchLite16 { static constexpr int T = 1; };

		struct ArchA2Base
		{
			static constexpr int NA = 1;
			static constexpr int NLA[2] = { 23, 0 };
			static constexpr int DIL[2][32] = { { 1, 3, 7, 17, 41, 101, 239, 1, 3, 7, 17, 41, 101, 239, 1, 13, 1, 3, 7, 17, 41, 101, 239 }, { 0 } };
			static constexpr int K(int, int l) { return (l == 14 || l == 15) ? 15 : 6; }
			static constexpr int HEADK = 16;
			static constexpr bool LEAKY = true;
			static constexpr int CHUNK = 16;
			static constexpr bool COARSE = true;
			static constexpr bool GUARDHIST = true;
			static constexpr bool FOLD = false;
			static constexpr int SKEW = 0;
			static constexpr bool COMPACT = false;
			static constexpr int NT_DIL = 100;
		};
		struct ArchA2Full : ArchA2Base { static constexpr int CH[2] = { 8, 0 }; static constexpr int T = 2; };
		struct ArchA2Lite : ArchA2Base { static constexpr int CH[2] = { 4, 0 }; static constexpr int T = 4; };

		struct FamStd { typedef ArchStd A0; typedef ArchStd A1; static constexpr int N = 1; };
		struct FamLite { typedef ArchLite A0; typedef ArchLite A1; static constexpr int N = 1; };
		struct FamLitePacked { typedef ArchLite A0; typedef ArchLite16 A1; static constexpr int N = 2; };
		struct FamA2 { typedef ArchA2Full A0; typedef ArchA2Lite A1; static constexpr int N = 2; };
		struct FamLite16T1 { typedef ArchLite16T1 A0; typedef ArchLite16T1 A1; static constexpr int N = 1; };

		enum TapClass { TAP_LDS = 0, TAP_HIST = 1, TAP_BOTH = 2 };

		template <class A>
		struct Tab
		{
			static constexpr int NA = A::NA;
			static constexpr int TotalLayers() { int n = 0; for (int a = 0; a < NA; a++) n += A::NLA[a]; return n; }
			static constexpr int NL = TotalLayers();
			static constexpr int NSTAGES = NL + NA + 1;
			static constexpr int ArrOf(int L) { int a = 0; while (L >= A::NLA[a]) { L -= A::NLA[a]; a++; } return a; }
			static constexpr int InArr(int L) { int a = 0; while (L >= A::NLA[a]) { L -= A::NLA[a]; a++; } return L; }
			static constexpr int Dil(int L) { return A::DIL[ArrOf(L)][InArr(L)]; }
			static constexpr int GPof(int a) { return A::CH[a] / 4; }
			static constexpr bool FirstOfArr(int L) { return InArr(L) == 0; }
			static constexpr bool LastOfArr(int L) { return InArr(L) == A::NLA[ArrOf(L)] - 1; }
			static constexpr int KS(int L) { return A::K(ArrOf(L), InArr(L)); }
			static constexpr bool Fold(int L) { return A::FOLD && KS(L) == 3 && GPof(ArrOf(L)) >= 2; }
			static constexpr int HEADK = A::HEADK;
			static constexpr int NRINGS = NL + (HEADK > 1 ? 1 : 0);
			static constexpr bool ExactRing(int L) { return L < NL && !FirstOfArr(L) && Dil(L) >= FRAMES && (KS(L) - 1) * Dil(L) >= 2 * FRAMES && ((KS(L) - 1) * Dil(L)) % 16 == 0; }
			static constexpr int HistFrames(int L) { return L < NL ? ((KS(L) - 1) * Dil(L) + 15) / 16 * 16 : (HEADK - 1 + 15) / 16 * 16; }
			static constexpr bool CompactRing(int L) { return A::COMPACT && L < NL && KS(L) > 1 && HistFrames(L) <= WN_COMPACT_MAX_HISTORY; }
			static constexpr int RingFrames(int L)
			{
				if (ExactRing(L)) return (KS(L) - 1) * Dil(L);
				if (CompactRing(L)) return 3 * HistFrames(L);
				return HistFrames(L) + FRAMES;
			}
			static constexpr int RingKeep(int L) { return ExactRing(L) ? RingFrames(L) : (CompactRing(L) ? HistFrames(L) : RingFrames(L) - FRAMES); }
			static constexpr int RingG(int L) { return GPof(L < NL ? ArrOf(L) : NA - 1); }
			static constexpr int RingOff(int L)
			{
				int o = WN_HEADER_F4;
				for (int l = 0; l < L; l++) o += RingFrames(l) * RingG(l);
				return o;
			}
			static constexpr int StateF4 = (RingOff(NRINGS) + 15) / 16 * 16;
			static constexpr int StageOfLayer(int L) { return 1 + L + ArrOf(L); }
			static constexpr int FirstLayerOfArr(int a) { int L = 0; for (int i = 0; i < a; i++) L += A::NLA[i]; return L; }
			static constexpr int LinkStage(int a) { return FirstLayerOfArr(a) + a; }
			static constexpr int LinkNC(int a) { const int Po = 4 / GPof(a - 1), Pn = 4 / GPof(a); return Po > Pn ? Po : Pn; }
			static constexpr int LayerOfStage(int s)
			{
				for (int L = 0; L < NL; L++)
					if (StageOfLayer(L) == s) return L;
				return -1;
			}
			static constexpr int StageOps(int s)
			{
				if (s == 0) return 1;
				if (s == NSTAGES - 1) return 2 * HEADK + 1;
				for (int a = 1; a < NA; a++)
					if (s == LinkStage(a)) return 4 * LinkNC(a) + 1;
				return 2 * KS(LayerOfStage(s)) + 4;
			}
			static constexpr int AOff(int s) { int o = 0; for (int i = 0; i < s; i++) o += StageOps(i) * 64; return o; }
			static constexpr int WsplitQuads = AOff(NSTAGES);
			static constexpr int CHUNK = A::CHUNK;
			static constexpr int TapOps(int s) { return s == NSTAGES - 1 ? 2 * HEADK : 2 * KS(LayerOfStage(s)); }
			static constexpr bool Chunked(int s) { return StageOps(s) > CHUNK; }
			static constexpr int TapChunks(int s) { return (TapOps(s) + CHUNK - 1) / CHUNK; }
			static constexpr int NumChunks(int s) { return Chunked(s) ? TapChunks(s) + 1 : 1; }
			static constexpr int ChunkBegin(int s, int c)
			{
				if (!Chunked(s)) return 0;
				if (c >= TapChunks(s)) return TapOps(s);
				const int pairs = TapOps(s) / 2, n = TapChunks(s);
				return 2 * ((pairs * c + n - 1) / n);
			}
			static constexpr int ChunkEnd(int s, int c) { return !Chunked(s) ? StageOps(s) : (c >= TapChunks(s) ? StageOps(s) : ChunkBegin(s, c + 1)); }
			static constexpr int ChunkIndex(int s, int c) { int n = 0; for (int i = 0; i < s; i++) n += NumChunks(i); return n + c; }
			static constexpr int MaxChunkOps()
			{
				int m = 0;
				for (int s = 0; s < NSTAGES; s++)
					for (int c = 0; c < NumChunks(s); c++) m = (ChunkEnd(s, c) - ChunkBegin(s, c)) > m ? (ChunkEnd(s, c) - ChunkBegin(s, c)) : m;
				return m;
			}
			static constexpr int MaxGP() { int m = 0; for (int a = 0; a < NA; a++) m = GPof(a) > m ? GPof(a) : m; return m; }
		};

		template <class A_, int NF_, int SPB_, bool PK_, bool COH_ = false, bool NT_ = false>
		struct Cfg
		{
			static constexpr bool COH = COH_;
			static constexpr bool NT = NT_;
			typedef A_ A;
			typedef Tab<A_> TB;
			static constexpr int NF = NF_, T = A_::T, FW = 16 * T, WPS = NF_ / FW, SPB = SPB_ * T / 2, NTHREADS = 64 * WPS * SPB;
			static_assert(WPS >= 1 && WPS * FW == NF_, "block length is a whole number of waves");
			static constexpr bool PK = PK_;
			static constexpr int MAXOPS = A_::CHUNK;
			static_assert(TB::MaxChunkOps() <= MAXOPS, "stage operand chunk");
			static constexpr int HPF = 5;
			static constexpr int SKEW = (SPB == 2 && !PK_ && T == 2 && A_::SKEW > 0) ? A_::SKEW : 0;
			static constexpr int NWB = SKEW > 0 ? SPB : 1;
			static constexpr int STG_THREADS = NTHREADS / NWB;
			static constexpr bool AUX16 = !PK_ && SKEW == 0;
			static constexpr int AUX_OFF = 0;
			static constexpr int IMG_OFF = AUX_OFF + SPB * FRAMES * (PK_ ? 32 : (AUX16 ? 16 : 8));
			static constexpr int IMG_ONE = TB::MaxGP() * PLANE * 16;
			static constexpr int WBUF_OFF = IMG_OFF + SPB * 2 * IMG_ONE;
			static constexpr int WBUF_ONE = MAXOPS * 1024;
			static constexpr int IDOP_OFF = WBUF_OFF + NWB * 2 * WBUF_ONE;
			static constexpr int DUMP_OFF = IDOP_OFF + 1024;
			static constexpr int FLAG_OFF = DUMP_OFF + 1024;
			static constexpr int BCAST_OFF = FLAG_OFF + 16 * SPB;
			static constexpr int LDS_BYTES = BCAST_OFF + (COH_ ? 64 : 0);
			static_assert(LDS_BYTES <= 80 * 1024, "two workgroups per CU");
		};

		template <int GP, int T>
		struct Geo
		{
			static_assert(GP == 4 || GP == 2 || GP == 1, "full lane modes of 16 / 8 / 4 channels");
			static constexpr int P = 4 / GP;
			static_assert(T % P == 0, "every tile slot of a set is a tile of the wave");
			static constexpr int S = T / P;
		};

		constexpr int TapClassOf(int F0, int P, int i, int shift)
		{
			const int lo = F0 + 16 * P * i - shift, hi = lo + 16 * P - 1;
			return hi < 0 ? TAP_HIST : (lo >= 0 ? TAP_LDS : TAP_BOTH);
		}

		template <class C, int RG>
		constexpr bool SmallRing() { return C::A::GUARDHIST && C::TB::RingKeep(RG) <= GUARD; }

		template <class C>
		constexpr int WaveTapClass(int w, int P, int i, int shift, bool small)
		{
			if (small) return TAP_LDS;
			if (!C::A::COARSE || w == 0 || C::WPS <= 2) return TapClassOf(C::FW * w, P, i, shift);
			const int first = TapClassOf(C::FW * 1, P, i, shift);
			for (int v = 2; v < C::WPS; v++)
				if (TapClassOf(C::FW * v, P, i, shift) != first) return TAP_BOTH;
			return first;
		}

		template <class C, int L>
		struct LayerSig
		{
			typedef typename C::TB TB;
			static constexpr int GP = TB::GPof(TB::ArrOf(L)), P = Geo<GP, C::T>::P, S = Geo<GP, C::T>::S, d = TB::Dil(L), K = TB::KS(L);
			static constexpr bool NEXT = !TB::LastOfArr(L);
			static constexpr int LN = NEXT ? L + 1 : L;
			static constexpr int dn = NEXT ? TB::Dil(LN) : 0, Kn = NEXT ? TB::KS(LN) : 1;
			static constexpr bool FOLD = TB::Fold(L) && !C::PK;
			static constexpr unsigned long long Of(int w)
			{
				unsigned long long s = 0;
				for (int k = 0; k < K - 1; k++)
					for (int i = 0; i < S; i++) s = s * 3 + (unsigned)WaveTapClass<C>(w, P, i, d * (K - 1 - k), SmallRing<C, L>());
				for (int k = 0; k < Kn - 1 && k < C::HPF; k++)
					for (int i = 0; i < S; i++) s = s * 3 + (unsigned)WaveTapClass<C>(w, P, i, dn * (Kn - 1 - k), SmallRing<C, LN>());
				return s;
			}
			static constexpr int Rep(int w) { int r = w; for (int v = w - 1; v >= 0; v--) if (Of(v) == Of(w)) r = v; return r; }
			static constexpr unsigned MaskOf(int r) { unsigned m = 0; for (int w = 0; w < C::WPS; w++) if (Rep(w) == r) m |= 1u << w; return m; }
			static constexpr bool LastRep(int r) { for (int w = r + 1; w < C::WPS; w++) if (Rep(w) == w) return false; return true; }
		};

		struct Ctx
		{
			__amdgpu_buffer_rsrc_t srsrc;
			__amdgpu_buffer_rsrc_t wrsrc;
			int myPos;
			int wave, sub, waveAll;
			int lane;
			int gs0, gs1;
			unsigned wbuf;
			int stgWave;
#ifdef NA_SP_TRACE
			long long* trace;
			int nwaves;
#endif
		};

#ifdef NA_SP_TRACE
#define SPK_STAMP(stage, point) do { __builtin_amdgcn_sched_barrier(0); if (cx.trace != nullptr && cx.lane == 0) cx.trace[(((stage) * 8 + (point)) * cx.nwaves) + cx.waveAll] = (long long)__builtin_readcyclecounter(); __builtin_amdgcn_sched_barrier(0); } while (0)
#else
#define SPK_STAMP(stage, point) (void)0
#endif

		template <class C, int GP>
		struct Lanes
		{
			int fl;
			int cg;
			unsigned img;
			unsigned aux;
			unsigned ring;
// ... 228 lines not shown
			static constexpr bool SAME = c + 1 < C::TB::NumChunks(s);
			static constexpr int S = SAME ? s : s + 1, CN = SAME ? c + 1 : 0;
			typedef Stager<C, S, CN> St;
		};

		template <class C>
		__device__ __forceinline__ u32x4 WOp(const Ctx& cx, int s, int c, int m)
		{
			const int buf = C::TB::ChunkIndex(s, c) & 1, local = m - C::TB::ChunkBegin(s, c);
			return LdsRead16(cx.wbuf + (unsigned)(buf * C::WBUF_ONE + ((NA_ABL & 128) ? 0 : local) * 1024) + (unsigned)cx.lane * 16u);
		}

		template <bool PACKED>
		__device__ __forceinline__ f32x4 ActivateTanh(f32x4 a)
		{
			if (PACKED)
			{
				const f32x2 lo = FastTanh2(f32x2{ a.x, a.y }), hi = FastTanh2(f32x2{ a.z, a.w });
				return f32x4{ lo.x, lo.y, hi.x, hi.y };
			}
			return f32x4{ FastTanh(a.x), FastTanh(a.y), FastTanh(a.z), FastTanh(a.w) };
		}

		template <class C, int GP>
		__device__ __forceinline__ u32x4 TapLds(const Ctx& cx, const Lanes<C, GP>& ln, int imgRead, int shift, int i, int cls)
		{
			constexpr int P = Geo<GP, C::T>::P;
			if (NA_ABL & 256) return u32x4{ (unsigned)shift, 0, 0, 0 };
			if (cls == TAP_LDS) return LdsRead16(ln.img + (unsigned)(imgRead * C::IMG_ONE) + (unsigned)((16 * P * i - shift) * 16));
			int off = C::FW * cx.wave + 16 * P * i + ln.fl - shift;
			off = off < -1 ? -1 : off;
			return LdsRead16((unsigned)(C::IMG_OFF + imgRead * C::IMG_ONE + GUARD * 16) + (unsigned)(cx.sub * 2 * C::IMG_ONE) + (unsigned)((ln.cg * PLANE + off) * 16));
		}

		template <class C, int RG, int GP, int WR>
		__device__ __forceinline__ f32x4 ConvTap(const Ctx& cx, const Lanes<C, GP>& ln, int imgRead, int shift, int i, u32x4 ah, u32x4 al, u32x4 hist, f32x4 acc)
		{
			constexpr int P = Geo<GP, C::T>::P;
			const int cls = WaveTapClass<C>(WR, P, i, shift, SmallRing<C, RG>());
			if (cls != TAP_LDS)
			{
				acc = Mfma(ah, hist, acc);
				acc = MfmaLo<1>(al, hist, acc);
			}
			if (cls != TAP_HIST)
			{
				const u32x4 b = TapLds<C, GP>(cx, ln, imgRead, shift, i, cls);
				acc = Mfma(ah, b, acc);
				acc = MfmaLo<1>(al, b, acc);
			}
			return acc;
		}

		template <class C, int RG, int GP, int WR>
		__device__ __forceinline__ f32x4 ConvTapFold(const Ctx& cx, const Lanes<C, GP>& ln, int imgRead, int shift, int i, u32x4 ah, u32x4 hist, f32x4 acc, u32x2& th)
		{
			constexpr int P = Geo<GP, C::T>::P;
			const int cls = WaveTapClass<C>(WR, P, i, shift, SmallRing<C, RG>());
			th = u32x2{ 0, 0 };
			if (cls != TAP_LDS)
			{
				acc = Mfma(ah, hist, acc);
				th = u32x2{ hist.x, hist.y };
			}
			if (cls != TAP_HIST)
			{
				const u32x4 b = TapLds<C, GP>(cx, ln, imgRead, shift, i, cls);
				acc = Mfma(ah, b, acc);
				th = cls == TAP_LDS ? u32x2{ b.x, b.y } : u32x2{ th.x | b.x, th.y | b.y };
			}
			return acc;
		}

		template <class C, int L, int WR, int c>
		__device__ __forceinline__ void LayerChunk(const Ctx& cx, const Lanes<C, C::TB::GPof(C::TB::ArrOf(L))>& ln, State& st, u32x4 (&ax)[LayerSig<C, L>::S],
			f32x4 (&acc)[LayerSig<C, L>::S])
		{
			typedef typename C::TB TB;
			typedef LayerSig<C, L> SG;
			constexpr int GP = SG::GP, S = SG::S, K = SG::K, s = TB::StageOfLayer(L), NCH = TB::NumChunks(s), CB = TB::ChunkBegin(s, c), CE = TB::ChunkEnd(s, c);
			constexpr int imgRead = s & 1, imgWrite = (s + 1) & 1, LN = SG::LN;
			constexpr bool LASTLAYER = TB::LastOfArr(L) && TB::ArrOf(L) == TB::NA - 1;
			constexpr int NEXTMINSHIFT = SG::NEXT ? TB::Dil(LN) : (1 << 20);
			constexpr bool OWN = 2 * (K - 1) >= CB && 2 * (K - 1) < CE;
			constexpr bool TAIL = 2 * K >= CB && 2 * K < CE;
			constexpr int LATER = ((OWN && SG::NEXT) ? HistLoadsOf<C, LN>() : 0) + ((TAIL && SG::NEXT && !LASTLAYER) ? StoresOf<C, LN>() : 0);
			typedef typename NextChunk<C, s, c>::St NextStager;
			if constexpr (c == 0)
			{
				if constexpr (SG::NEXT) GuardStage<C, LN, GP>(cx, ln, imgWrite);
				else if constexpr (LASTLAYER && TB::HEADK > 1) GuardStage<C, TB::NL, GP>(cx, ln, (TB::NSTAGES - 1 + 1) & 1);
			}
			NextStager::Begin(cx);
			if constexpr (c == 0)
			{
#pragma unroll
				for (int i = 0; i < S; i++) ax[i] = AuxRead<C, GP>(ln, i);
			}
			constexpr int KLO = CB / 2, KHI = (CE / 2 < K - 1) ? CE / 2 : K - 1;
			constexpr int NX = (KHI > C::HPF) ? KHI - (KLO > C::HPF ? KLO : C::HPF) : 0;
			u32x4 hx[NX > 0 ? NX : 1][S];
#pragma unroll
			for (int k = KLO; k < KHI; k++)
			{
				if (k < C::HPF) continue;
#pragma unroll
				for (int i = 0; i < S; i++)
					if (WaveTapClass<C>(WR, SG::P, i, ShiftOf<C, L>(k), SmallRing<C, L>()) != TAP_LDS) hx[k - (KLO > C::HPF ? KLO : C::HPF)][i] = HistLoadAt<C, L, WR>(cx, ln.ring, ln.fl, ShiftOf<C, L>(k), i);
			}
			static_assert(!SG::FOLD || (NCH == 1 && K == 3), "folded operands: K = 3 layers in one chunk");
			u32x2 th[SG::FOLD ? 2 : 1][S];
#pragma unroll
			for (int k = KLO; k < KHI; k++)
			{
				const u32x4 ah = WOp<C>(cx, s, c, 2 * k), al = SG::FOLD ? ah : WOp<C>(cx, s, c, 2 * k + 1);
#pragma unroll
				for (int i = 0; i < S; i++)
				{
					u32x4 h = u32x4{ 0, 0, 0, 0 };
					if (WaveTapClass<C>(WR, SG::P, i, ShiftOf<C, L>(k), SmallRing<C, L>()) != TAP_LDS)
						h = (k < C::HPF) ? st.hist[k < C::HPF ? k : 0][i] : hx[k >= C::HPF ? k - (KLO > C::HPF ? KLO : C::HPF) : 0][i];
					if constexpr (SG::FOLD) acc[i] = ConvTapFold<C, L, GP, WR>(cx, ln, imgRead, ShiftOf<C, L>(k), i, ah, h, acc[i], th[k < 2 ? k : 0][i]);
					else acc[i] = ConvTap<C, L, GP, WR>(cx, ln, imgRead, ShiftOf<C, L>(k), i, ah, al, h, acc[i]);
				}
			}
			if constexpr (SG::FOLD)
			{
				const u32x4 al01 = WOp<C>(cx, s, c, 1);
#pragma unroll
				for (int i = 0; i < S; i++) acc[i] = Mfma(al01, u32x4{ th[0][i].x, th[0][i].y, th[1][i].x, th[1][i].y }, acc[i]);
			}
			if constexpr (OWN)
			{
				if constexpr (SG::NEXT) HistPrefetch<C, LN, WR>(cx, ln.ring, ln.fl, st);
				const u32x4 ah = WOp<C>(cx, s, c, 2 * K - 2), al = WOp<C>(cx, s, c, 2 * K - 1);
#pragma unroll
				for (int i = 0; i < S; i++)
				{
					acc[i] = Mfma(ah, st.xs[i], acc[i]);
					if constexpr (SG::FOLD) acc[i] = Mfma(al, u32x4{ st.xs[i].x, st.xs[i].y, ax[i].x, ax[i].y }, acc[i]);
					else acc[i] = MfmaLo<1>(al, st.xs[i], acc[i]);
				}
			}
			if constexpr (TAIL)
			{
				if constexpr (!SG::FOLD)
				{
					const u32x4 xa = WOp<C>(cx, s, c, 2 * K);
#pragma unroll
					for (int i = 0; i < S; i++) acc[i] = Mfma(xa, ax[i], acc[i]);
				}
				SPK_STAMP(s, 1);
				f32x4 z[S];
#pragma unroll
				for (int i = 0; i < S; i++)
				{
					if constexpr (C::A::LEAKY) z[i] = f32x4{ LeakyReLU(acc[i].x), LeakyReLU(acc[i].y), LeakyReLU(acc[i].z), LeakyReLU(acc[i].w) };
					else z[i] = ActivateTanh<(NA_PK_TANH != 0) && (C::NTHREADS < 512)>(acc[i]);
				}
				SPK_STAMP(s, 2);
				const u32x4 idop = LdsRead16((unsigned)C::IDOP_OFF + (unsigned)cx.lane * 16u);
				const u32x4 w1h = WOp<C>(cx, s, c, 2 * K + 1), w1l = WOp<C>(cx, s, c, 2 * K + 2), b1a = SG::FOLD ? w1l : WOp<C>(cx, s, c, 2 * K + 3);
#pragma unroll
				for (int i = 0; i < S; i++)
				{
					const u32x4 zs = SplitQuad(z[i]);
					st.hd[i] = Mfma(idop, zs, st.hd[i]);
					if constexpr (!LASTLAYER)
					{
						f32x4 y = st.xc[i];
						y = Mfma(w1h, zs, y);
						const u32x4 axi = NA_SPK_AUX2 ? AuxRead<C, GP>(ln, i) : ax[i];
						if constexpr (SG::FOLD) y = Mfma(w1l, u32x4{ zs.x, zs.y, axi.x, axi.y }, y);
						else
						{
							y = MfmaLo<2>(w1l, zs, y);
							y = Mfma(b1a, axi, y);
						}
						st.xc[i] = y;
						if constexpr (SG::NEXT)
						{
							st.xs[i] = Split<C>(y, cx);
							Publish<C, LN, GP, NEXTMINSHIFT>(cx, ln, st.xs[i], i, imgWrite);
						}
					}
				}
				SPK_STAMP(s, 3);
			}
			NextStager::template End<LATER>();
			SPK_STAMP(s, 4);
			BlockBarrier<C::NTHREADS / 64>();
			if constexpr (c + 1 < NCH) LayerChunk<C, L, WR, c + 1>(cx, ln, st, ax, acc);
		}

		template <class C, int L, int WR>
		__device__ __forceinline__ void LayerBody(const Ctx& cx, const Lanes<C, C::TB::GPof(C::TB::ArrOf(L))>& ln, State& st)
		{
			constexpr int S = LayerSig<C, L>::S;
			SPK_STAMP(C::TB::StageOfLayer(L), 0);
			u32x4 ax[S];
			f32x4 acc[S];
#pragma unroll
			for (int i = 0; i < S; i++) acc[i] = f32x4{ 0.0f, 0.0f, 0.0f, 0.0f };
			LayerChunk<C, L, WR, 0>(cx, ln, st, ax, acc);
			SPK_STAMP(C::TB::StageOfLayer(L), 5);
		}

		template <class C, int L, int W>
		__device__ __forceinline__ void LayerDispatch(const Ctx& cx, const Lanes<C, C::TB::GPof(C::TB::ArrOf(L))>& ln, State& st)
		{
			typedef LayerSig<C, L> SG;
			if constexpr (W < C::WPS)
			{
				if constexpr (SG::Rep(W) != W) LayerDispatch<C, L, W + 1>(cx, ln, st);
				else if constexpr (SG::LastRep(W)) LayerBody<C, L, W>(cx, ln, st);
				else
				{
					constexpr unsigned MASK = SG::MaskOf(W);
					if ((MASK >> cx.wave) & 1u) LayerBody<C, L, W>(cx, ln, st);
					else LayerDispatch<C, L, W + 1>(cx, ln, st);
				}
			}
		}

		template <class C, int L, int W>
		__device__ __forceinline__ void FirstHistDispatch(const Ctx& cx, unsigned laneRing, int fl, State& st)
		{
			typedef typename C::TB TB;
			constexpr int GP = TB::GPof(TB::ArrOf(L)), P = Geo<GP, C::T>::P, S = Geo<GP, C::T>::S;
			if constexpr (W < C::WPS)
			{
				constexpr bool same = [] {
					bool r = true;
					for (int w = W + 1; w < C::WPS; w++)
						for (int k = 0; k < PrefetchTaps<C, L>(); k++)
							for (int i = 0; i < S; i++) r = r && WaveTapClass<C>(w, P, i, ShiftOf<C, L>(k), SmallRing<C, L>()) == WaveTapClass<C>(W, P, i, ShiftOf<C, L>(k), SmallRing<C, L>());
					return r;
				}();
				if constexpr (same) HistPrefetch<C, L, W>(cx, laneRing, fl, st);
				else
				{
					if (cx.wave == W) HistPrefetch<C, L, W>(cx, laneRing, fl, st);
					else FirstHistDispatch<C, L, W + 1>(cx, laneRing, fl, st);
				}
			}
// ... 243 lines not shown
			if constexpr (PK)
			{
				for (int i = wave * 64 + lane; i < FRAMES; i += C::WPS * 64)
				{
					float c[4];
#pragma unroll
					for (int q = 0; q < 4; q++) c[q] = (rowOf[q] >= 0 && i < NF) ? LoadIn<C::COH>(in + (size_t)rowOf[q] * inStride + i) : 0.0f;
#pragma unroll
					for (int q = 0; q < 4; q++)
					{
						const float cc = ClampCond(c[q], ga.condLimit);
						const _Float16 ch = (_Float16)cc, cl = (_Float16)(cc - (float)ch);
						const f16x2 a = { ch, (_Float16)1.0f }, b = { cl, (_Float16)1.0f };
						*reinterpret_cast<__attribute__((address_space(3))) u32x2*>((LdsPtr)(size_t)(unsigned)(C::AUX_OFF + ((sub * 4 + q) * FRAMES + i) * 8)) =
							u32x2{ __builtin_bit_cast(unsigned, a), __builtin_bit_cast(unsigned, b) };
					}
				}
			}
			else
			{
				for (int i = wave * 64 + lane; i < FRAMES; i += C::WPS * 64)
				{
					const float c = (i < NF) ? ClampCond(LoadIn<C::COH>(in + (size_t)row * inStride + i), ga.condLimit) : 0.0f;
					const _Float16 ch = (_Float16)c, cl = (_Float16)(c - (float)ch);
					const f16x2 a = { ch, (_Float16)1.0f }, b = { cl, (_Float16)1.0f }, d = { ch, (_Float16)0.0f };
					if constexpr (C::AUX16)
						LdsWrite16((unsigned)(C::AUX_OFF + (sub * FRAMES + i) * 16), u32x4{ __builtin_bit_cast(unsigned, a), __builtin_bit_cast(unsigned, b), __builtin_bit_cast(unsigned, d), 0u });
					else
						*reinterpret_cast<__attribute__((address_space(3))) u32x2*>((LdsPtr)(size_t)(unsigned)(C::AUX_OFF + (sub * FRAMES + i) * 8)) =
							u32x2{ __builtin_bit_cast(unsigned, a), __builtin_bit_cast(unsigned, b) };
				}
			}
			for (int i = tid; i < SPB * 2 * TB::MaxGP(); i += C::NTHREADS) LdsWrite16((unsigned)(C::IMG_OFF + (i * PLANE + GUARD - 1) * 16), u32x4{ 0, 0, 0, 0 });
			if (tid < 64)
			{
				const int i = lane & 15, q = lane >> 4;
				const unsigned one = 0x3c00u;
				const unsigned lo = (q == (i >> 2)) ? (((i & 3) == 0) ? one : ((i & 3) == 1) ? (one << 16) : 0u) : 0u;
				const unsigned hi = (q == (i >> 2)) ? (((i & 3) == 2) ? one : ((i & 3) == 3) ? (one << 16) : 0u) : 0u;
				LdsWrite16((unsigned)C::IDOP_OFF + (unsigned)lane * 16u, u32x4{ lo, hi, lo, hi });
			}
			if constexpr (C::A::LEAKY)
			{
				if (tid < SPB) *reinterpret_cast<__attribute__((address_space(3))) unsigned*>((LdsPtr)(size_t)(unsigned)(C::FLAG_OFF + 16 * tid)) = 0u;
			}
			if (cx.stgWave == 0) LdsWrite16(cx.wbuf + (unsigned)lane * 16u, BufLoad(cx.wrsrc, lane * 16));
			BlockBarrier<C::NTHREADS / 64>();

			if constexpr (C::SKEW > 0)
			{
				if (sub != 0)
					for (int k = 0; k < C::SKEW; k++) BlockBarrier<C::NTHREADS / 64>();
			}
			State st;
			RunArrays<C, 0>(cx, st, out, (size_t)row * outStride, outRow, pack, ga.headScale, live);
			if constexpr (C::SKEW > 0)
			{
				if (sub == 0)
					for (int k = 0; k < C::SKEW; k++) BlockBarrier<C::NTHREADS / 64>();
			}

#ifdef NA_SP_TRACE
			if (cx.trace != nullptr && lane == 0) cx.trace[((C::TB::NSTAGES * 8 + 1) * cx.nwaves) + waveAll] = (long long)__builtin_readcyclecounter();
#endif
			if constexpr (C::A::LEAKY)
			{
				BlockBarrier<C::NTHREADS / 64>();
				if (wave == 0) CountRangeEvent(header, (int)*reinterpret_cast<__attribute__((address_space(3))) unsigned*>((LdsPtr)(size_t)(unsigned)(C::FLAG_OFF + 16 * sub)), lane, live);
			}
			if (wave == 0 && live && lane < ga.nrings)
			{
				const int R = ga.ringFrames[lane];
				int p = cx.myPos + NF;
				if (p >= R) p -= R;
				if (p >= R) p -= R;
				if (p >= R) p -= R;
				header[lane] = p;
			}
		}

#ifndef NA_SPK_OCC
#define NA_SPK_OCC(nf, spb) (((nf) * (spb) / 64) < 1 ? 1 : ((nf) * (spb) / 64))
#endif
		template <class F, int NF, int SPB>
		constexpr int OccOf() { return F::A0::T == 1 ? (NA_SPK_OCC(NF, SPB) / 2 < 1 ? 1 : NA_SPK_OCC(NF, SPB) / 2) : NA_SPK_OCC(NF, SPB); }
		template <class F, int NF, int SPB, bool PK, bool NT = false>
		__global__ void __launch_bounds__(64 * (NF / (16 * F::A0::T)) * (SPB * F::A0::T / 2)) __attribute__((amdgpu_waves_per_eu(OccOf<F, NF, SPB>()))) WaveNetSpecKernel(const LaunchArgs args,
			const float* __restrict__ in, float* __restrict__ out, long inStride, long outStride
#ifdef NA_SP_TRACE
			, long long* __restrict__ trace, int traceBlock
#endif
			)
		{
			typedef Cfg<typename F::A0, NF, SPB, PK, false, NT> C;
			typedef Cfg<typename F::A1, NF, SPB, PK, false, NT> C1;
			static_assert(C::NTHREADS == C1::NTHREADS, "members of a family launch the same workgroup");
			extern __shared__ __attribute__((aligned(16))) char dynSmem[];
			asm volatile("" : : "s"((unsigned)(size_t)(LdsPtr)dynSmem));

			int gi = 0;
			for (int i = 1; i < args.numGroups; i++)
				if ((int)blockIdx.x >= args.g[i].firstBlock) gi = i;
			const GroupArgs& ga = args.g[gi];
			const int groupBlock = (int)blockIdx.x - ga.firstBlock;
#if NA_SPK_DELAY > 0
			if (blockIdx.x >= gridDim.x / 2)
				for (int k = 0; k < NA_SPK_DELAY; k += 100) __builtin_amdgcn_s_sleep(100);
#endif
#ifdef NA_SP_TRACE
			long long* tr = ((int)blockIdx.x == traceBlock) ? trace : nullptr;
			if (F::N > 1 && ga.arch == 1) RunWorkgroup<C1>(ga, groupBlock, in, out, inStride, outStride, tr);
			else RunWorkgroup<C>(ga, groupBlock, in, out, inStride, outStride, tr);
#else
			if (F::N > 1 && ga.arch == 1) RunWorkgroup<C1>(ga, groupBlock, in, out, inStride, outStride);
			else RunWorkgroup<C>(ga, groupBlock, in, out, inStride, outStride);
#endif
		}

		template <class F, int NF, int SPB, bool PK>
		__global__ void __launch_bounds__(64 * (NF / (16 * F::A0::T)) * (SPB * F::A0::T / 2)) __attribute__((amdgpu_waves_per_eu(OccOf<F, NF, SPB>()))) WaveNetSpecResidentKernel(const LaunchArgs args,
			const ResidentArgs ra
#ifdef NA_SP_TRACE
			, long long* __restrict__ trace, int traceBlock
#endif
			)
		{
			typedef Cfg<typename F::A0, NF, SPB, PK, true> C;
			typedef Cfg<typename F::A1, NF, SPB, PK, true> C1;
			static_assert(C::NTHREADS == C1::NTHREADS && C::BCAST_OFF == C1::BCAST_OFF, "members of a family launch the same workgroup");
			extern __shared__ __attribute__((aligned(16))) char dynSmem[];
			asm volatile("" : : "s"((unsigned)(size_t)(LdsPtr)dynSmem));
			typedef __attribute__((address_space(3))) unsigned long long* Lds64;
			Lds64 const bc = reinterpret_cast<Lds64>((LdsPtr)(size_t)(unsigned)C::BCAST_OFF);
			if (threadIdx.x == 0)
			{
				bc[5] = ra.base + ra.wgDone[blockIdx.x];
				bc[6] = ~0ull;
				if (ra.startDelay > 0 && 2 * blockIdx.x >= gridDim.x)
				{
					const unsigned long long t0 = __builtin_amdgcn_s_memrealtime();
					while (__builtin_amdgcn_s_memrealtime() - t0 < ra.startDelay) __builtin_amdgcn_s_sleep(16);
				}
			}
			for (;;)
			{
				if (threadIdx.x == 0)
				{
					int z = 0;
					asm volatile("" : "+v"(z));
					const ResidentArgs& r = (&ra)[__builtin_amdgcn_readfirstlane(z)];
					unsigned long long k = bc[5];
					long blk = (long)bc[6];
					unsigned long long go = 1;
					if (blk >= 0) blk += (long)gridDim.x;
					if (blk < 0 || blk >= (long)r.numBlocks)
					{
						const bool finished = blk >= 0;
						if (finished) k++;
						const unsigned slot = (unsigned)(k % RESIDENT_RING);
						if (finished) __hip_atomic_store(&r.wgDone[blockIdx.x], (unsigned)(k - r.base), __ATOMIC_RELAXED, __HIP_MEMORY_SCOPE_AGENT);
						const ResidentCmd* cmd = &r.ctrl->cmd[(k + 1) % RESIDENT_RING];
						auto word = [](const void* p) { return __hip_atomic_load(reinterpret_cast<const unsigned long long*>(p), __ATOMIC_RELAXED, __HIP_MEMORY_SCOPE_SYSTEM); };
						unsigned long long cIn = word(&cmd->in), cOut = word(&cmd->out), cIs = word(&cmd->inStride), cOs = word(&cmd->outStride);
						unsigned long long cSeq = word(&cmd->seq), cChk = word(&cmd->check);
						if (finished)
						{
							const unsigned before = __hip_atomic_fetch_add(&r.doneCount[slot], 1u, __ATOMIC_RELAXED, __HIP_MEMORY_SCOPE_AGENT);
							if (before == gridDim.x - 1)
							{
								__hip_atomic_store(&r.doneCount[slot], 0u, __ATOMIC_RELAXED, __HIP_MEMORY_SCOPE_AGENT);
								__hip_atomic_store(&r.status->completed, k, __ATOMIC_RELAXED, __HIP_MEMORY_SCOPE_SYSTEM);
							}
						}
						const unsigned long long t0 = __builtin_amdgcn_s_memrealtime();
						bool leaving = false;
						while (cSeq != k + 1 || cChk != ResidentCmdCheck(cIn, cOut, cIs, cOs, cSeq))
						{
							if (leaving) { go = 0; break; }
							leaving = word(&r.ctrl->exitAfter) <= k || __builtin_amdgcn_s_memrealtime() - t0 > r.idleTicks;
// ... 109 lines not shown
				a.arch = (F::N > 1 && (m.spec_arch == WN_SPEC_LITE16 || m.spec_arch == WN_SPEC_A2LITE)) ? 1 : 0;
				const int c0 = a.arch == 1 ? F::A1::CH[0] : F::A0::CH[0], c1 = a.arch == 1 ? F::A1::CH[1] : F::A0::CH[1];
				a.gps0 = std::max(1, c0 / 4 / a.pack);
				a.gps1 = (a.pack > 1 && c1 < 4 * a.pack) ? 0 : std::max(1, c1 / 4 / a.pack);
				if (a.pack > 1 && !PK) return hipErrorInvalidValue;
				if (PK && g.slots == nullptr) return hipErrorInvalidValue;
				const int spbArch = a.arch == 1 ? C1::SPB : C::SPB;
				blocks += (g.numStreams + spbArch - 1) / spbArch;
			}
			*blocksOut = blocks;
			return hipSuccess;
		}

		template <class F, int NF, int SPB, bool PK>
		static hipError_t FillLaunchArgs(const WnFrameGroup* groups, int numGroups, LaunchArgs& args, int* blocksOut)
		{
			args = {};
			args.numGroups = numGroups;
			return FillGroupArgs<F, NF, SPB, PK>(groups, numGroups, args.g, blocksOut);
		}

		template <class F, int NF, int SPB, bool PK>
		__global__ void __launch_bounds__(64 * (NF / (16 * F::A0::T)) * (SPB * F::A0::T / 2)) __attribute__((amdgpu_waves_per_eu(OccOf<F, NF, SPB>()))) WaveNetSpecTableKernel(
			const GroupArgs* __restrict__ table, int numGroups, const float* __restrict__ in, float* __restrict__ out, long inStride, long outStride)
		{
			typedef Cfg<typename F::A0, NF, SPB, PK> C;
			typedef Cfg<typename F::A1, NF, SPB, PK> C1;
			extern __shared__ __attribute__((aligned(16))) char dynSmem[];
			asm volatile("" : : "s"((unsigned)(size_t)(LdsPtr)dynSmem));
			typedef const __attribute__((address_space(4))) GroupArgs* TablePtr;
			TablePtr tab = (TablePtr)(size_t)table;
			int lo = 0, hi = numGroups - 1;
			while (lo < hi)
			{
				const int mid = (lo + hi + 1) >> 1;
				if (tab[mid].firstBlock <= (int)blockIdx.x) lo = mid;
				else hi = mid - 1;
			}
			GroupArgs ga;
			{
				const auto& e = tab[lo];
				ga.stages = e.stages; ga.wsplit = e.wsplit; ga.ringFrames = e.ringFrames; ga.state = e.state; ga.slots = e.slots; ga.rows = e.rows;
				ga.nstages = e.nstages; ga.nrings = e.nrings; ga.stateF4 = e.stateF4; ga.wsplitQuads = e.wsplitQuads;
				ga.headScale = e.headScale;
				ga.numStreams = e.numStreams; ga.slot0 = e.slot0; ga.row0 = e.row0;
				ga.maxG = e.maxG; ga.firstBlock = e.firstBlock; ga.pack = e.pack; ga.condLimit = e.condLimit; ga.arch = e.arch;
				ga.gps0 = e.gps0; ga.gps1 = e.gps1; ga.saturate = e.saturate;
			}
			const int groupBlock = (int)blockIdx.x - ga.firstBlock;
#ifdef NA_SP_TRACE
			if (F::N > 1 && ga.arch == 1) RunWorkgroup<C1>(ga, groupBlock, in, out, inStride, outStride, nullptr);
			else RunWorkgroup<C>(ga, groupBlock, in, out, inStride, outStride, nullptr);
#else
			if (F::N > 1 && ga.arch == 1) RunWorkgroup<C1>(ga, groupBlock, in, out, inStride, outStride);
			else RunWorkgroup<C>(ga, groupBlock, in, out, inStride, outStride);
#endif
		}

		template <class F, int NF, int SPB, bool PK>
		static hipError_t LaunchTable(const WnFrameGroup* groups, int numGroups, const float* in, float* out, long inStride, long outStride, hipStream_t stream, WnLaunchTable& t)
		{
			typedef Cfg<typename F::A0, NF, SPB, PK> C;
			typedef Cfg<typename F::A1, NF, SPB, PK> C1;
			std::vector<GroupArgs> fresh((size_t)numGroups);
			int blocks = 0;
			const hipError_t fe = FillGroupArgs<F, NF, SPB, PK>(groups, numGroups, fresh.data(), &blocks);
			if (fe != hipSuccess) return fe;
			const void* dev = nullptr;
			const hipError_t ee = t.Ensure(fresh.data(), fresh.size() * sizeof(GroupArgs), stream, &dev);
			if (ee != hipSuccess) return ee;
			if (t.prepareOnly) return hipSuccess;
			constexpr int LDS_BYTES = C::LDS_BYTES > C1::LDS_BYTES ? C::LDS_BYTES : C1::LDS_BYTES;
			if (LDS_BYTES > 64 * 1024)
			{
				static PerDeviceOnce attr;
				const hipError_t e = attr.Run([] { return hipFuncSetAttribute(reinterpret_cast<const void*>(WaveNetSpecTableKernel<F, NF, SPB, PK>), hipFuncAttributeMaxDynamicSharedMemorySize, LDS_BYTES); });
				if (e != hipSuccess) return e;
			}
			hipLaunchKernelGGL((WaveNetSpecTableKernel<F, NF, SPB, PK>), dim3((unsigned)blocks), dim3(C::NTHREADS), LDS_BYTES, stream,
				reinterpret_cast<const GroupArgs*>(dev), numGroups, in, out, inStride, outStride);
			return hipGetLastError();
		}

		template <class F, int NF, int SPB, bool PK, bool NT = false>
		static hipError_t Launch(const WnFrameGroup* groups, int numGroups, const float* in, float* out, long inStride, long outStride, hipStream_t stream)
		{
			typedef Cfg<typename F::A0, NF, SPB, PK> C;
			typedef Cfg<typename F::A1, NF, SPB, PK> C1;
			LaunchArgs args;
			int blocks = 0;
			const hipError_t fe = FillLaunchArgs<F, NF, SPB, PK>(groups, numGroups, args, &blocks);
			if (fe != hipSuccess) return fe;
			constexpr int LDS_BYTES = C::LDS_BYTES > C1::LDS_BYTES ? C::LDS_BYTES : C1::LDS_BYTES;
			if (LDS_BYTES > 64 * 1024)
			{
				static PerDeviceOnce attr;
				const hipError_t e = attr.Run([] { return hipFuncSetAttribute(reinterpret_cast<const void*>(WaveNetSpecKernel<F, NF, SPB, PK, NT>), hipFuncAttributeMaxDynamicSharedMemorySize, LDS_BYTES); });
				if (e != hipSuccess) return e;
			}
			hipLaunchKernelGGL((WaveNetSpecKernel<F, NF, SPB, PK, NT>), dim3((unsigned)blocks), dim3(C::NTHREADS), LDS_BYTES, stream, args, in, out, inStride, outStride
#ifdef NA_SP_TRACE
				, GetWaveNetTraceBuffer(), Tuning::Get().traceBlock
#endif
				);
			return hipGetLastError();
		}

		template <class F, int NF, int SPB, bool PK>
		static hipError_t LaunchResident(const WnFrameGroup* groups, int numGroups, ResidentArgs ra, hipStream_t stream, int* gridOut)
		{
			typedef Cfg<typename F::A0, NF, SPB, PK, true> C;
			typedef Cfg<typename F::A1, NF, SPB, PK, true> C1;
			LaunchArgs args;
			int blocks = 0;
			const hipError_t fe = FillLaunchArgs<F, NF, SPB, PK>(groups, numGroups, args, &blocks);
			if (fe != hipSuccess) return fe;
			constexpr int LDS_BYTES = C::LDS_BYTES > C1::LDS_BYTES ? C::LDS_BYTES : C1::LDS_BYTES;
			static PerDeviceOnce attr;
			static std::atomic<int> perCU[kMaxHipDevices];
			int device = 0;
			hipError_t e = hipGetDevice(&device);
			if (e != hipSuccess) return e;
			if (device < 0 || device >= kMaxHipDevices) return hipErrorInvalidDevice;
			e = attr.Run([device] {
				hipError_t r = hipSuccess;
				if (LDS_BYTES > 64 * 1024)
					r = hipFuncSetAttribute(reinterpret_cast<const void*>(WaveNetSpecResidentKernel<F, NF, SPB, PK>), hipFuncAttributeMaxDynamicSharedMemorySize, LDS_BYTES);
				if (r != hipSuccess) return r;
				int nb = 0;
				r = hipOccupancyMaxActiveBlocksPerMultiprocessor(&nb, reinterpret_cast<const void*>(WaveNetSpecResidentKernel<F, NF, SPB, PK>), C::NTHREADS, LDS_BYTES);
				perCU[device].store(nb);
				return r;
			});
			if (e != hipSuccess) return e;
			const int resident = perCU[device].load() * CurrentDeviceCUs();
			int grid = std::min(blocks, resident);
			if (Tuning::Get().residentGrid > 0) grid = std::min(grid, Tuning::Get().residentGrid);
			*gridOut = grid;
			if (grid < 1) return hipErrorInvalidValue;
			if (stream == nullptr) return hipSuccess;
			ra.numBlocks = blocks;
			hipLaunchKernelGGL((WaveNetSpecResidentKernel<F, NF, SPB, PK>), dim3((unsigned)grid), dim3(C::NTHREADS), LDS_BYTES, stream, args, ra
#ifdef NA_SP_TRACE
				, GetWaveNetTraceBuffer(), Tuning::Get().traceBlock
#endif
				);
			return hipGetLastError();
		}

		template <class F, bool PK>
		static hipError_t LaunchNF(const WnFrameGroup* groups, int numGroups, const float* in, float* out, long inStride, long outStride, int n, int spb, hipStream_t stream,
			bool beyondCache = false)
		{
#ifdef NA_SP_QUICK
			(void)spb; (void)n; (void)beyondCache;
			return Launch<F, 128, 2, PK>(groups, numGroups, in, out, inStride, outStride, stream);
#else
			if constexpr (F::A0::T != 1)
				if (beyondCache && n == 128 && spb >= 2) return Launch<F, 128, 2, PK, true>(groups, numGroups, in, out, inStride, outStride, stream);
			if constexpr (F::A0::T == 1)
			{
				if (n == 128) return Launch<F, 128, 2, PK>(groups, numGroups, in, out, inStride, outStride, stream);
				if (n == 64) return Launch<F, 64, 2, PK>(groups, numGroups, in, out, inStride, outStride, stream);
				return Launch<F, 32, 2, PK>(groups, numGroups, in, out, inStride, outStride, stream);
			}
			else
			{
			if (n == 128) return spb >= 2 ? Launch<F, 128, 2, PK>(groups, numGroups, in, out, inStride, outStride, stream) : Launch<F, 128, 1, PK>(groups, numGroups, in, out, inStride, outStride, stream);
			if (n == 64) return spb >= 2 ? Launch<F, 64, 2, PK>(groups, numGroups, in, out, inStride, outStride, stream) : Launch<F, 64, 1, PK>(groups, numGroups, in, out, inStride, outStride, stream);
			if constexpr (F::A0::T == 2 && F::A1::T == 2)
				return spb >= 2 ? Launch<F, 32, 2, PK>(groups, numGroups, in, out, inStride, outStride, stream) : Launch<F, 32, 1, PK>(groups, numGroups, in, out, inStride, outStride, stream);
			else return hipErrorNotSupported;
			}
#endif
		}

		hipError_t LaunchSpecLite(const WnFrameGroup* groups, int numGroups, const float* in, float* out, long inStride, long outStride, int n, int spb, bool packed,
			hipStream_t stream, bool oneTilePerWave = false, bool beyondCache = false);
		hipError_t LaunchSpecA2(const WnFrameGroup* groups, int numGroups, const float* in, float* out, long inStride, long outStride, int n, int spb, hipStream_t stream,
			bool beyondCache = false);
		hipError_t LaunchSpecA2Table(const WnFrameGroup* groups, int numGroups, const float* in, float* out, long inStride, long outStride, int n, int spb, hipStream_t stream,
			WnLaunchTable& table);
		hipError_t LaunchSpecLiteTable(const WnFrameGroup* groups, int numGroups, const float* in, float* out, long inStride, long outStride, int n, int spb, bool packed,
// ... 4 lines not shown
```

neuralaudio_amd/csrc/wavenet_spec_kernels.hip:

```cpp
#include "wavenet_spec_impl.h"

namespace na
{
	static int& SpecSwitch()
	{
		static int on = Tuning::Get().wnSpecOff ? 0 : 1;
		return on;
	}
	bool WaveNetSpecEnabled() { return SpecSwitch() != 0; }
	void SetWaveNetSpecEnabled(bool on) { SpecSwitch() = on ? 1 : 0; }

	int WaveNetSpecArchId(const WnSplitStage* stages, int nstages, int stateF4, int wsplitQuads)
	{
		if (spk::Matches<spk::ArchStd>(stages, nstages, stateF4, wsplitQuads)) return WN_SPEC_STD;
		if (spk::Matches<spk::ArchLite>(stages, nstages, stateF4, wsplitQuads)) return WN_SPEC_LITE;
		if (spk::Matches<spk::ArchLite16>(stages, nstages, stateF4, wsplitQuads)) return WN_SPEC_LITE16;
		if (spk::Matches<spk::ArchA2Full>(stages, nstages, stateF4, wsplitQuads)) return WN_SPEC_A2FULL;
		if (spk::Matches<spk::ArchA2Lite>(stages, nstages, stateF4, wsplitQuads)) return WN_SPEC_A2LITE;
		return WN_SPEC_NONE;
	}

	hipError_t LaunchWaveNetSpecTable(const WnFrameGroup* groups, int numGroups, const float* in, float* out, long inStride, long outStride, int n,
		hipStream_t stream, WnLaunchTable& table)
	{
#ifdef NA_SP_QUICK
		return hipErrorNotSupported;
#else
		if (numGroups <= WN_FRAME_MAX_GROUPS || (n != 128 && n != 64) || !WaveNetSpecEnabled() || Tuning::Get().spSpb > 0) return hipErrorNotSupported;
		const int arch = groups[0].model->spec_arch;
		const bool lite = arch == WN_SPEC_LITE || arch == WN_SPEC_LITE16, a2 = arch == WN_SPEC_A2FULL || arch == WN_SPEC_A2LITE;
		if (arch != WN_SPEC_STD && !lite && !a2) return hipErrorNotSupported;
		bool packed = false;
		long streams = 0, slots2 = 0;
		for (int i = 0; i < numGroups; i++)
		{
			const int a = groups[i].model->spec_arch;
			const bool same = lite ? (a == WN_SPEC_LITE || a == WN_SPEC_LITE16) : (a2 ? (a == WN_SPEC_A2FULL || a == WN_SPEC_A2LITE) : a == WN_SPEC_STD);
			if (groups[i].numStreams <= 0 || !same) return hipErrorNotSupported;
			packed = packed || groups[i].pack > 1;
			const int per2 = a == WN_SPEC_A2LITE ? 4 : 2;
			streams += groups[i].numStreams;
			slots2 += (groups[i].numStreams + per2 - 1) / per2 * per2;
		}
		if (!lite && packed) return hipErrorNotSupported;
		if (packed)
			for (int i = 0; i < numGroups; i++)
				if (groups[i].slots == nullptr) return hipErrorNotSupported;
		if (!packed)
			for (int i = 0; i < numGroups; i++)
				if (groups[i].model->spec_arch == WN_SPEC_LITE16) return hipErrorNotSupported;
		const int spb = (slots2 * 4 > streams * 5) ? 1 : 2;
		if (a2) return spk::LaunchSpecA2Table(groups, numGroups, in, out, inStride, outStride, n, spb, stream, table);
		if (!lite)
		{
			if (n == 64) return spb == 2 ? spk::LaunchTable<spk::FamStd, 64, 2, false>(groups, numGroups, in, out, inStride, outStride, stream, table)
										 : spk::LaunchTable<spk::FamStd, 64, 1, false>(groups, numGroups, in, out, inStride, outStride, stream, table);
			return spb == 2 ? spk::LaunchTable<spk::FamStd, 128, 2, false>(groups, numGroups, in, out, inStride, outStride, stream, table)
							: spk::LaunchTable<spk::FamStd, 128, 1, false>(groups, numGroups, in, out, inStride, outStride, stream, table);
		}
		return spk::LaunchSpecLiteTable(groups, numGroups, in, out, inStride, outStride, n, spb, packed, stream, table);
#endif
	}

	hipError_t LaunchWaveNetSpecFused(const WnFrameGroup* groups, int numGroups, const float* in, float* out, long inStride, long outStride, int n,
		hipStream_t stream, int sharing)
	{
		if (numGroups <= 0 || numGroups > WN_FRAME_MAX_GROUPS || (n != 128 && n != 64 && n != 32)) return hipErrorNotSupported;
		if (!WaveNetSpecEnabled()) return hipErrorNotSupported;
		const int arch = groups[0].model->spec_arch;
		if (arch == WN_SPEC_NONE) return hipErrorNotSupported;
		auto familyOf = [](int a) { return (a == WN_SPEC_LITE || a == WN_SPEC_LITE16) ? 1 : ((a == WN_SPEC_A2FULL || a == WN_SPEC_A2LITE) ? 2 : 0); };
		const int fam = familyOf(arch);
		bool packed = false, lite16 = false;
		for (int i = 0; i < numGroups; i++)
		{
			const int a = groups[i].model->spec_arch;
			if (groups[i].numStreams <= 0 || a == WN_SPEC_NONE || familyOf(a) != fam || (fam == 0 && a != arch)) return hipErrorNotSupported;
			packed = packed || groups[i].pack > 1;
			lite16 = lite16 || a == WN_SPEC_LITE16;
		}
		if (packed)
			for (int i = 0; i < numGroups; i++)
				if (groups[i].slots == nullptr) return hipErrorNotSupported;
		const int spbEnv = Tuning::Get().spSpb;
		const int residentHalf = 2 * CurrentDeviceCUs();
		int halfGroups = 0;
		for (int i = 0; i < numGroups; i++)
		{
			const int per = groups[i].model->spec_arch == WN_SPEC_A2LITE ? 2 : 1;
			halfGroups += (groups[i].numStreams + per - 1) / per;
		}
		const bool beyondCache = (sharing & WN_SHARING_BEYOND_CACHE) != 0;
		sharing &= ~WN_SHARING_BEYOND_CACHE;
		const int spb = spbEnv > 0 ? spbEnv : (halfGroups * std::max(sharing, 1) > residentHalf ? 2 : 1);
#ifdef NA_SP_QUICK
		if (arch != WN_SPEC_STD || packed) return hipErrorNotSupported;
		return spk::LaunchNF<spk::FamStd, false>(groups, numGroups, in, out, inStride, outStride, n, spb, stream);
#else
		if (fam == 0) return packed ? hipErrorNotSupported : spk::LaunchNF<spk::FamStd, false>(groups, numGroups, in, out, inStride, outStride, n, spb, stream, beyondCache);
		if (fam == 2) return packed ? hipErrorNotSupported : spk::LaunchSpecA2(groups, numGroups, in, out, inStride, outStride, n, spb, stream, beyondCache);
		if (!packed && lite16) return hipErrorNotSupported;
		const bool noT1 = Tuning::Get().spNoT1;
		bool all16 = packed && !noT1;
		int virtualStreams = 0;
		for (int i = 0; i < numGroups; i++)
		{
			all16 = all16 && groups[i].model->spec_arch == WN_SPEC_LITE16;
			virtualStreams += groups[i].numStreams;
		}
		const bool t1 = all16 && spbEnv == 0 && virtualStreams <= CurrentDeviceCUs();
		return spk::LaunchSpecLite(groups, numGroups, in, out, inStride, outStride, n, spb, packed, stream, t1, beyondCache);
#endif
	}
}
```

neuralaudio_amd/csrc/wavenet_split_kernels.hip:

```cpp
#include "device_once.h"
#include "tuning.h"
#include <algorithm>
#include <cstddef>
#include <cstdlib>

#include <hip/hip_runtime.h>

#include "wavenet_dev.h"
#include "wavenet_launch.h"

#include "wavenet_split_dev.h"

namespace na
{
	namespace sp
	{
#ifdef NA_SP_TRACE
#define SP_STAMP(point) do { __builtin_amdgcn_sched_barrier(0); if (cx.trace != nullptr && cx.lane == 0) cx.trace[((s * 8 + (point)) * cx.nwaves) + cx.waveAll] = (long long)__builtin_readcyclecounter(); __builtin_amdgcn_sched_barrier(0); } while (0)
#else
#define SP_STAMP(point) (void)0
#endif
		struct Stage
		{
			int type, flags, G, Gp, ksize, dilation, ring_off, ring_frames, ring_id, out_ring_off, out_ring_frames, out_ring_id, out_G, a_off, a_ops, reserved;
// ... 141 lines not shown
		__device__ __forceinline__ u32x4 SplitOf(const Ctx& cx, State<T>& st, f32x4 v)
		{
			if (cx.saturate) return SplitQuadSatLoose(v, st.hit);
			return SplitQuad(v);
		}

		__device__ __forceinline__ int OpaqueLane(const Ctx& cx)
		{
			int lane = cx.lane;
			asm volatile("" : "+v"(lane));
			return lane;
		}

		template <int GP, int T>
		__device__ __forceinline__ void FrameOf(const Ctx& cx, int lane, int s, int& f, int& cg, bool& tileLive)
		{
			constexpr int P = Geo<GP, T>::P;
			const int q = lane >> 4;
			const int p = q / GP;
			cg = q % GP;
			f = cx.F0 + 16 * (P * s + p) + (lane & 15);
			tileLive = !Geo<GP, T>::PARTIAL || (P * s + p < T);
		}

		template <bool PK>
		__device__ __forceinline__ u32x4 AuxOf(const Ctx& cx, int f, int cg, int gsShift)
		{
			if constexpr (PK)
			{
				if (gsShift < 0)
				{
					const u32x2 v = cx.auxp[(2 * cg) * FRAMES + (f & (FRAMES - 1))], w = cx.auxp[(2 * cg + 1) * FRAMES + (f & (FRAMES - 1))];
					return u32x4{ v.x, v.y, (v.x & 0xffffu) | (w.x << 16), (w.y & 0xffffu) | (w.x << 16) };
				}
				const u32x2 v = cx.auxp[(cg >> gsShift) * FRAMES + (f & (FRAMES - 1))];
				return u32x4{ v.x, v.y, v.x & 0xffffu, 0u };
			}
			else return cx.auxq[f & (FRAMES - 1)];
		}

		template <int GP, int T, int NTHREADS, int HPF, bool GEN, bool PK>
		__device__ __forceinline__ void RunLayers(const Ctx& cx, int& s, Stage& sd, int& cur, State<T>& st)
		{
			constexpr int S = Geo<GP, T>::S;
			constexpr int P = Geo<GP, T>::P;
			const WeightStager<NTHREADS, GEN> stager;
			const int lane = OpaqueLane(cx);
			int f[S], cg[S];
			bool live[S];
#pragma unroll
			for (int i = 0; i < S; i++) FrameOf<GP, T>(cx, lane, i, f[i], cg[i], live[i]);

			u32x4 hist[HPF][S];
			{
				const int pos0 = __builtin_amdgcn_readlane(cx.myPos, sd.ring_id);
#pragma unroll
				for (int t = 0; t < HPF; t++)
#pragma unroll
					for (int i = 0; i < S; i++)
						hist[t][i] = LoadHistory(cx, sd.ring_off, sd.ring_frames, sd.G, pos0, f[i], cg[i], sd.dilation * (sd.ksize - 1 - t), t < sd.ksize - 1 && cg[i] < sd.G);
			}
			do
			{
				Stage sdn = sd;
				sdn.a_ops = 0;
				sdn.type = -1;
				if (s + 1 < cx.nstages) sdn = LoadStage(cx.stages, s + 1);
				SP_STAMP(0);
				stager.Begin(cx, (s + 1) & 1, sdn);
				SP_STAMP(6);
				const u32x4* wl = cx.wbuf + (s & 1) * cx.wstride + lane;
				const u32x4* imgCur = cx.img + cur * cx.imgStride;
				u32x4* imgNext = cx.img + (cur ^ 1) * cx.imgStride;
				const int K = GEN ? sd.ksize : 3, d = sd.dilation, G = GEN ? sd.G : GP;
				const bool mask = GEN && (Geo<GP, T>::PARTIAL || G < GP);
				const int inPos0 = __builtin_amdgcn_readlane(cx.myPos, sd.ring_id);
				const int outPos0 = (sd.out_ring_id >= 0) ? RingAdvance(__builtin_amdgcn_readlane(cx.myPos, sd.out_ring_id), cx.n, sd.out_ring_frames) : 0;
				const int gsShift = PK ? (sd.reserved == 0 ? -1 : (sd.reserved >> 1)) : 0;

				f32x4 acc[S];
#pragma unroll
				for (int i = 0; i < S; i++) acc[i] = f32x4{ 0.0f, 0.0f, 0.0f, 0.0f };
				const bool fold = GP >= 2 && (sd.flags & WN_FLAG_FOLD) != 0;
				u32x2 th[2][S];
#pragma unroll
				for (int k = 0; k < HPF; k++)
				{
					if (!GEN || k < K - 1)
					{
						const u32x4 ah = wl[WOP(2 * k)], al = wl[WOP(2 * k + 1)];
						const int shift = d * (K - 1 - k);
						const int lo = cx.F0 - shift, hi = cx.F0 + 16 * P * S - 1 - shift;
						if (hi < 0)
						{
#pragma unroll
							for (int i = 0; i < S; i++)
							{
								acc[i] = Mfma(ah, hist[k][i], acc[i]);
								if (fold) th[k < 2 ? k : 0][i] = u32x2{ hist[k][i].x, hist[k][i].y };
								else acc[i] = MfmaLo<1>(al, hist[k][i], acc[i]);
							}
						}
						else if (lo >= 0)
						{
#pragma unroll
							for (int i = 0; i < S; i++)
							{
								u32x4 b = imgCur[ImgIdx(cg[i], f[i] - shift)];
								if (mask) b = (live[i] && cg[i] < G) ? b : u32x4{ 0, 0, 0, 0 };
								acc[i] = Mfma(ah, b, acc[i]);
								if (fold) th[k < 2 ? k : 0][i] = u32x2{ b.x, b.y };
								else acc[i] = MfmaLo<1>(al, b, acc[i]);
							}
						}
						else
						{
#pragma unroll
							for (int i = 0; i < S; i++)
							{
								u32x4 b = TapInBlock(imgCur, f[i] - shift, cg[i]);
								if (mask) b = (live[i] && cg[i] < G) ? b : u32x4{ 0, 0, 0, 0 };
								acc[i] = Mfma(ah, hist[k][i], acc[i]);
								if (!fold) acc[i] = MfmaLo<1>(al, hist[k][i], acc[i]);
								acc[i] = Mfma(ah, b, acc[i]);
								if (fold) th[k < 2 ? k : 0][i] = u32x2{ hist[k][i].x | b.x, hist[k][i].y | b.y };
								else acc[i] = MfmaLo<1>(al, b, acc[i]);
							}
						}
					}
				}
				if (HPF >= 2 && fold)
				{
					const u32x4 al01 = wl[WOP(1)];
#pragma unroll
					for (int i = 0; i < S; i++) acc[i] = Mfma(al01, u32x4{ th[0][i].x, th[0][i].y, th[1][i].x, th[1][i].y }, acc[i]);
				}
				SP_STAMP(7);
				{
					const bool haveNext = (s + 1 < cx.nstages) && sdn.type == WN_ST_LAYER && sdn.Gp == GP;
					const int nextPos0 = __builtin_amdgcn_readlane(cx.myPos, haveNext ? sdn.ring_id : 0);
#pragma unroll
					for (int t = 0; t < HPF; t++)
#pragma unroll
						for (int i = 0; i < S; i++)
							hist[t][i] = LoadHistory(cx, sdn.ring_off, sdn.ring_frames, sdn.G, nextPos0, f[i], cg[i], sdn.dilation * (sdn.ksize - 1 - t),
								haveNext && t < sdn.ksize - 1 && cg[i] < sdn.G);
				}
				if constexpr (GEN)
				for (int k = HPF; k < K - 1; k++)
				{
					const u32x4 ah = wl[WOP(2 * k)], al = wl[WOP(2 * k + 1)];
					const int shift = d * (K - 1 - k);
#pragma unroll
					for (int i = 0; i < S; i++)
					{
						const int lo = cx.F0 + 16 * P * i - shift;
						u32x4 b = TapOperandInline(cx, imgCur, sd.ring_off, sd.ring_frames, G, inPos0, f[i], cg[i] < G ? cg[i] : 0, shift, lo, lo + 16 * P - 1);
						if (mask) b = (live[i] && cg[i] < G) ? b : u32x4{ 0, 0, 0, 0 };
						acc[i] = Mfma(ah, b, acc[i]);
						if (fold) th[k < 2 ? k : 0][i] = u32x2{ b.x, b.y };
						else acc[i] = MfmaLo<1>(al, b, acc[i]);
					}
				}
				if (HPF < 2 && fold)
				{
					const u32x4 al01 = wl[WOP(1)];
#pragma unroll
					for (int i = 0; i < S; i++) acc[i] = Mfma(al01, u32x4{ th[0][i].x, th[0][i].y, th[1][i].x, th[1][i].y }, acc[i]);
				}
				{
					const u32x4 ah = wl[WOP(2 * K - 2)], al = wl[WOP(2 * K - 1)], xa = wl[WOP(2 * K)];
#pragma unroll
					for (int i = 0; i < S; i++)
					{
						u32x4 b = imgCur[ImgIdx(cg[i], f[i])];
						if (mask) b = (live[i] && cg[i] < G) ? b : u32x4{ 0, 0, 0, 0 };
						const u32x4 ax = AuxOf<PK>(cx, f[i], cg[i], gsShift);
						acc[i] = Mfma(ah, b, acc[i]);
						if (fold) acc[i] = Mfma(al, u32x4{ b.x, b.y, ax.x, ax.y }, acc[i]);
						else
						{
							acc[i] = MfmaLo<1>(al, b, acc[i]);
							acc[i] = Mfma(xa, ax, acc[i]);
						}
					}
				}

				SP_STAMP(1);
				f32x4 z[S];
				if (sd.flags & WN_FLAG_LEAKY)
				{
#pragma unroll
					for (int i = 0; i < S; i++) z[i] = f32x4{ LeakyReLU(acc[i].x), LeakyReLU(acc[i].y), LeakyReLU(acc[i].z), LeakyReLU(acc[i].w) };
				}
				else if (sd.flags & WN_FLAG_STD_TANH)
				{
#pragma unroll
					for (int i = 0; i < S; i++) z[i] = f32x4{ StdTanh(acc[i].x), StdTanh(acc[i].y), StdTanh(acc[i].z), StdTanh(acc[i].w) };
				}
				else
				{
#pragma unroll
					for (int i = 0; i < S; i++)
					{
						if (NA_PK_TANH)
						{
							const f32x2 lo = FastTanh2(f32x2{ acc[i].x, acc[i].y }), hi = FastTanh2(f32x2{ acc[i].z, acc[i].w });
							z[i] = f32x4{ lo.x, lo.y, hi.x, hi.y };
						}
						else z[i] = f32x4{ FastTanh(acc[i].x), FastTanh(acc[i].y), FastTanh(acc[i].z), FastTanh(acc[i].w) };
					}
				}
				SP_STAMP(2);
				const bool pub = (sd.flags & WN_FLAG_PUBLISH) != 0;
				const u32x4 idop = cx.idop[lane];
				{
					const u32x4 w1h = wl[WOP(2 * K + 1)], w1l = wl[WOP(2 * K + 2)], b1a = wl[WOP(2 * K + 3)];
#pragma unroll
					for (int i = 0; i < S; i++)
					{
						const u32x4 zs = SplitQuad(z[i]);
						const u32x4 ax = AuxOf<PK>(cx, f[i], cg[i], gsShift);
						st.hd[i] = Mfma(idop, zs, st.hd[i]);
						f32x4 y = st.xc[i];
						y = Mfma(w1h, zs, y);
						if (fold) y = Mfma(w1l, u32x4{ zs.x, zs.y, ax.x, ax.y }, y);
						else
						{
							y = MfmaLo<2>(w1l, zs, y);
							y = Mfma(b1a, ax, y);
						}
						st.xc[i] = y;
						Publish(cx, imgNext, SplitOf(cx, st, y), f[i], cg[i], pub && (!GEN || (live[i] && cg[i] < sd.out_G)), sd.out_ring_off, sd.out_ring_frames, sd.out_G, outPos0,
							pub ? cx.nSt : 0);
					}
				}
				if (sd.flags & WN_FLAG_PUBLISH) cur ^= 1;
				SP_STAMP(3);
				stager.template End<(HPF + 1) * S>(cx, (s + 1) & 1, sdn);
				SP_STAMP(4);
				BlockBarrier<NTHREADS / 64>();
				SP_STAMP(5);
				sd = sdn;
				s++;
			} while (s < cx.nstages && sd.type == WN_ST_LAYER && sd.Gp == GP);
		}

		template <int GP, int T, int NTHREADS, bool GEN, bool PK>
		__device__ __forceinline__ void RechannelStage(const Ctx& cx, int& s, Stage& sd, int& cur, State<T>& st)
		{
			constexpr int S = Geo<GP, T>::S;
			const WeightStager<NTHREADS, GEN> stager;
			const int lane = OpaqueLane(cx);
			Stage sdn = LoadStage(cx.stages, s + 1);
			SP_STAMP(0);
			stager.Begin(cx, (s + 1) & 1, sdn);
			const u32x4* wl = cx.wbuf + (s & 1) * cx.wstride + lane;
			u32x4* imgNext = cx.img + (cur ^ 1) * cx.imgStride;
			const int outPos0 = RingAdvance(__builtin_amdgcn_readlane(cx.myPos, sd.out_ring_id), cx.n, sd.out_ring_frames);
			const u32x4 ra = wl[0];
#pragma unroll
			for (int i = 0; i < S; i++)
			{
				int f, cg; bool live;
				FrameOf<GP, T>(cx, lane, i, f, cg, live);
				const u32x4 ax = AuxOf<PK>(cx, f, cg, PK ? (sd.reserved >> 1) : 0);
				f32x4 x = f32x4{ 0.0f, 0.0f, 0.0f, 0.0f };
				x = Mfma(ra, ax, x);
				st.xc[i] = x;
				st.hd[i] = f32x4{ 0.0f, 0.0f, 0.0f, 0.0f };
				Publish(cx, imgNext, SplitOf(cx, st, x), f, cg, live && cg < sd.out_G, sd.out_ring_off, sd.out_ring_frames, sd.out_G, outPos0, cx.nSt);
			}
			cur ^= 1;
			SP_STAMP(1); SP_STAMP(2); SP_STAMP(3);
			stager.template End<0>(cx, (s + 1) & 1, sdn);
			SP_STAMP(4);
			BlockBarrier<NTHREADS / 64>();
			SP_STAMP(5);
			sd = sdn;
			s++;
		}

		template <int GPO, int GPN, int T, int NTHREADS, bool GEN, bool PK>
		__device__ __forceinline__ void LinkStage(const Ctx& cx, int& s, Stage& sd, int& cur, State<T>& st)
		{
			constexpr int Po = 4 / GPO, Pn = 4 / GPN, NC = Po > Pn ? Po : Pn;
			constexpr int So = Geo<GPO, T>::S, Sn = Geo<GPN, T>::S;
			const WeightStager<NTHREADS, GEN> stager;
			const int lane = OpaqueLane(cx);
			Stage sdn = LoadStage(cx.stages, s + 1);
			SP_STAMP(0);
			stager.Begin(cx, (s + 1) & 1, sdn);
			const u32x4* wl = cx.wbuf + (s & 1) * cx.wstride + lane;
			u32x4* imgNext = cx.img + (cur ^ 1) * cx.imgStride;
			const int outPos0 = RingAdvance(__builtin_amdgcn_readlane(cx.myPos, sd.out_ring_id), cx.n, sd.out_ring_frames);

			u32x4 hs[So], xs[So];
#pragma unroll
			for (int i = 0; i < So; i++)
			{
// ... 395 lines not shown
```

Measured before the change: 3698.

## Compact folded-layer weight blocks and add opt-in four-workgroup quad spec kernel

```diff
diff --git a/include/neuralaudio_amd.h b/include/neuralaudio_amd.h
--- a/include/neuralaudio_amd.h
+++ b/include/neuralaudio_amd.h
@@ -179,6 +179,8 @@
 NA_EXTERN int NA_DebugClassifyNam(const char* jsonText);
 NA_EXTERN int NA_DebugPackedWeights(NeuralModel* model, int* packFactor, float* out, int capacity);
 NA_EXTERN int NA_DebugSplitPlan(NeuralModel* model, int* stages, int stageCapacity, unsigned short* wsplit, long long wsplitCapacity, long long* wsplitCount);
+NA_EXTERN int NA_DebugSplitPlanCompact(NeuralModel* model, int* stages, int stageCapacity, unsigned short* wsplit, long long wsplitCapacity, long long* wsplitCount);
+NA_EXTERN int NA_DebugSplitSpecArch(NeuralModel* model, int out[6]);
 NA_EXTERN void NA_DebugSetWaveNetSpec(int on);
 NA_EXTERN int NA_DebugSetRecurrentQuadMin(int streams);
 NA_EXTERN long long NA_DebugRecurrentQuadLaunches(void);
diff --git a/neuralaudio_amd/capi.py b/neuralaudio_amd/capi.py
--- a/neuralaudio_amd/capi.py
+++ b/neuralaudio_amd/capi.py
@@ -20,7 +20,7 @@
     "NA_BatchSetQuality", "NA_BatchGetActiveSubModel", "NA_BatchPrewarm", "NA_BatchProcess", "NA_BatchProcessDevice",
     "NA_BatchSynchronize", "NA_BatchGetHipStream", "NA_BatchAlgorithmicBytesPerSample", "NA_BatchMacsPerSample",
     "NA_BatchStateBytes", "NA_BatchStreamPackFactor", "NA_BatchStreamKernelName", "NA_DebugSetTraceBuffer", "NA_DebugSetWaveNetSpec", "NA_DebugSetRecurrentQuadMin", "NA_DebugRecurrentQuadLaunches", "NA_RegisterHostBuffer", "NA_UnregisterHostBuffer", "NA_BatchStreamInputLimit", "NA_BatchRemoveStreams", "NA_MultiCreate", "NA_MultiDestroy", "NA_MultiAddStreams", "NA_MultiCommit", "NA_MultiNumStreams", "NA_MultiNumShards", "NA_MultiShardRange", "NA_MultiProcess", "NA_MultiSubmit", "NA_MultiCollect", "NA_MultiSetQuality", "NA_ShardByCost", "NA_ModelStreamCost", "NA_BatchNumLiveStreams", "NA_BatchIsLive", "NA_SetWaveNetMathMode", "NA_SetLSTMMathMode", "NA_SetCompositeModelLoadMode",
-    "NA_IsQualityChangeRealtimeSafe", "NA_ProcessChecked", "NA_BatchSubmit", "NA_BatchCollect", "NA_BatchNextInput", "NA_BatchOutputView", "NA_BatchIsQualityChangeRealtimeSafe", "NA_DebugClassifyNam", "NA_DebugPackedWeights", "NA_DebugSplitPlan", "NA_ModelKernelInfo", "NA_BatchStreamRangeEvents", "NA_MultiSetFanIn", "NA_MultiGatheredOutput", "NA_RcclAvailable",
+    "NA_IsQualityChangeRealtimeSafe", "NA_ProcessChecked", "NA_BatchSubmit", "NA_BatchCollect", "NA_BatchNextInput", "NA_BatchOutputView", "NA_BatchIsQualityChangeRealtimeSafe", "NA_DebugClassifyNam", "NA_DebugPackedWeights", "NA_DebugSplitPlan", "NA_DebugSplitPlanCompact", "NA_DebugSplitSpecArch", "NA_ModelKernelInfo", "NA_BatchStreamRangeEvents", "NA_MultiSetFanIn", "NA_MultiGatheredOutput", "NA_RcclAvailable",
     "NA_BatchMarkTime", "NA_BatchWaitMarks", "NA_BatchElapsedMs", "NA_BatchUsesHalfLaunches", "NA_DebugSetRcclApi", "NA_BatchWaitOutputs", "NA_BatchUsesResidentLaunch", "NA_BatchSetResidentLaunch",
     "NA_BatchSetWaitLimitMs", "NA_BatchGetWaitLimitMs", "NA_BatchIsBroken", "NA_DebugStallDevice",
     "NA_RenderOffline", "NA_RenderPlan",
@@ -241,6 +241,8 @@
         "NA_MultiSetResampling": (C.c_int, [vp, C.c_int, C.c_int, C.c_int, C.c_int]),
         "NA_MultiGetResampleInfo": (C.c_int, [vp, C.POINTER(NA_ResampleInfo)]),
         "NA_DebugSplitPlan": (C.c_int, [vp, C.POINTER(C.c_int), C.c_int, C.POINTER(C.c_ushort), C.c_longlong, C.POINTER(C.c_longlong)]),
+        "NA_DebugSplitPlanCompact": (C.c_int, [vp, C.POINTER(C.c_int), C.c_int, C.POINTER(C.c_ushort), C.c_longlong, C.POINTER(C.c_longlong)]),
+        "NA_DebugSplitSpecArch": (C.c_int, [vp, C.POINTER(C.c_int)]),
     }
     for name, (res, args) in sig.items():
         try:
diff --git a/neuralaudio_amd/csrc/capi.cpp b/neuralaudio_amd/csrc/capi.cpp
--- a/neuralaudio_amd/csrc/capi.cpp
+++ b/neuralaudio_amd/csrc/capi.cpp
@@ -304,20 +304,48 @@
 #endif
 
 #ifndef NA_RELEASE
-int NA_DebugSplitPlan(NeuralModel* model, int* stages, int stageCapacity, unsigned short* wsplit, long long wsplitCapacity, long long* wsplitCount)
+static int DebugSplitPlan(const char* who, bool compactFold, NeuralModel* model, int* stages, int stageCapacity, unsigned short* wsplit, long long wsplitCapacity,
+	long long* wsplitCount)
 {
 	int r = -1;
 	Guard([&] {
 		NeuralAudio::GpuModel* gm = model ? dynamic_cast<NeuralAudio::GpuModel*>(model->model) : nullptr;
-		if (!gm) throw std::runtime_error("NA_DebugSplitPlan: not a model of this library");
+		if (!gm) throw std::runtime_error(std::string(who) + ": not a model of this library");
 		const auto& lm = gm->GetLoadedModel();
-		if (lm->subModels.size() != 1 || lm->subModels[0].desc->kind != na::MODEL_WAVENET) throw std::runtime_error("NA_DebugSplitPlan: not a WaveNet");
-		const na::WaveNetPlan plan = na::BuildWaveNetPlan(lm->subModels[0].desc->wavenet, true);
+		if (lm->subModels.size() != 1 || lm->subModels[0].desc->kind != na::MODEL_WAVENET) throw std::runtime_error(std::string(who) + ": not a WaveNet");
+		const na::WaveNetPlan plan = na::BuildWaveNetPlan(lm->subModels[0].desc->wavenet, true, compactFold);
 		static_assert(sizeof(na::WnSplitStage) == 16 * sizeof(int), "16 ints per stage");
 		r = (int)plan.sstages.size();
 		if (stages) memcpy(stages, plan.sstages.data(), sizeof(na::WnSplitStage) * (size_t)std::min(r, stageCapacity));
 		if (wsplitCount) *wsplitCount = (long long)plan.wsplit.size();
 		if (wsplit) memcpy(wsplit, plan.wsplit.data(), sizeof(uint16_t) * (size_t)std::min<long long>((long long)plan.wsplit.size(), wsplitCapacity));
+	});
+	return r;
+}
+int NA_DebugSplitPlan(NeuralModel* model, int* stages, int stageCapacity, unsigned short* wsplit, long long wsplitCapacity, long long* wsplitCount)
+{
+	return DebugSplitPlan("NA_DebugSplitPlan", false, model, stages, stageCapacity, wsplit, wsplitCapacity, wsplitCount);
+}
+int NA_DebugSplitPlanCompact(NeuralModel* model, int* stages, int stageCapacity, unsigned short* wsplit, long long wsplitCapacity, long long* wsplitCount)
+{
+	return DebugSplitPlan("NA_DebugSplitPlanCompact", true, model, stages, stageCapacity, wsplit, wsplitCapacity, wsplitCount);
+}
+#endif
+
+#ifndef NA_RELEASE
+int NA_DebugSplitSpecArch(NeuralModel* model, int out[6])
+{
+	int r = -1;
+	Guard([&] {
+		NeuralAudio::GpuModel* gm = model ? dynamic_cast<NeuralAudio::GpuModel*>(model->model) : nullptr;
+		if (!gm || !out) throw std::runtime_error("NA_DebugSplitSpecArch: not a model of this library");
+		const auto& lm = gm->GetLoadedModel();
+		if (lm->subModels.size() != 1 || lm->subModels[0].desc->kind != na::MODEL_WAVENET) throw std::runtime_error("NA_DebugSplitSpecArch: not a WaveNet");
+		const na::WaveNetPlan plan = na::BuildWaveNetPlan(lm->subModels[0].desc->wavenet, true);
+		out[1] = (int)(plan.wsplit.size() / 8);
+		out[0] = na::WaveNetSpecArchId(plan.sstages.data(), (int)plan.sstages.size(), plan.stateF4, out[1]);
+		na::WaveNetSpecStdTables(out + 2);
+		r = 0;
 	});
 	return r;
 }
diff --git a/neuralaudio_amd/csrc/tuning.cpp b/neuralaudio_amd/csrc/tuning.cpp
--- a/neuralaudio_amd/csrc/tuning.cpp
+++ b/neuralaudio_amd/csrc/tuning.cpp
@@ -32,6 +32,7 @@
 			t.wnDense = Int("NA_WN_DENSE", -1);
 			t.spT = Int("NA_SP_T", 0);
 			t.spSpb = Int("NA_SP_SPB", 0);
+			t.spQuad = Int("NA_SP_QUAD", -1);
 			t.spGen = Has("NA_SP_GEN");
 			t.wnSpecOff = IsZero("NA_WN_SPEC") || Has("NA_SP_T") || Has("NA_SP_GEN");
 			t.spNoT1 = Has("NA_SP_NO_T1");
diff --git a/neuralaudio_amd/csrc/tuning.h b/neuralaudio_amd/csrc/tuning.h
--- a/neuralaudio_amd/csrc/tuning.h
+++ b/neuralaudio_amd/csrc/tuning.h
@@ -13,6 +13,7 @@
 		bool wnSpecOff = false;
 		int spT = 0;
 		int spSpb = 0;
+		int spQuad = -1;
 		bool spGen = false;
 		bool spNoT1 = false;
 		bool spReverse = false;
diff --git a/neuralaudio_amd/csrc/wavenet_dev.h b/neuralaudio_amd/csrc/wavenet_dev.h
--- a/neuralaudio_amd/csrc/wavenet_dev.h
+++ b/neuralaudio_amd/csrc/wavenet_dev.h
@@ -79,6 +79,10 @@
 	};
 	static_assert(sizeof(WnSplitStage) == 64, "split stage descriptors are 64-byte records");
 
+	constexpr int WN_FOLD_OPS = 7;
+	constexpr int WnFoldSlot(int m) { return m - (m > 3 ? 1 : 0) - (m > 6 ? 1 : 0); }
+	constexpr bool WnFoldDead(int m) { return m == 3 || m == 6 || m == 9; }
+
 	constexpr int WN_GENERIC_MAX_CHANNELS = 128;
 	constexpr int WN_COL_STRIDE = 128;
 
diff --git a/neuralaudio_amd/csrc/wavenet_launch.h b/neuralaudio_amd/csrc/wavenet_launch.h
--- a/neuralaudio_amd/csrc/wavenet_launch.h
+++ b/neuralaudio_amd/csrc/wavenet_launch.h
@@ -137,6 +137,7 @@
 	bool WaveNetSpecEnabled();
 	void SetWaveNetSpecEnabled(bool on);
 	int WaveNetSpecArchId(const WnSplitStage* stages, int nstages, int stateF4, int wsplitQuads);
+	void WaveNetSpecStdTables(int out[4]);
 
 	hipError_t LaunchWaveNetGeneric(const WnPrewarmLayer* layers, int numLayers, const float* weights, const int* ringOffF4, const int* ringFrames,
 		const int* ringG, int nrings, int stateF4, int maxChannels, float headScale, float condLimit, bool saturate, float* state, const int* slots, const int* rows,
diff --git a/neuralaudio_amd/csrc/wavenet_plan.cpp b/neuralaudio_amd/csrc/wavenet_plan.cpp
--- a/neuralaudio_amd/csrc/wavenet_plan.cpp
+++ b/neuralaudio_amd/csrc/wavenet_plan.cpp
@@ -125,6 +125,7 @@
 
 			int pack = 1;
 			bool foldOk = false;
+			bool compactFold = true;
 			bool exactRings = false;
 			bool compactOk = false;
 
@@ -421,6 +422,32 @@
 						e[4] = wch; e[5] = w1h; e[6] = wch; e[7] = w1l;
 						e2[4] = wcl;
 					}
+			}
+
+			void CompactFoldedBlocks()
+			{
+				std::vector<uint16_t> image;
+				image.reserve(plan.wsplit.size());
+				for (WnSplitStage& st : plan.sstages)
+				{
+					const bool fold = st.type == WN_ST_LAYER && (st.flags & WN_FLAG_FOLD) != 0;
+					const int op0 = st.a_off / 64, first = (int)(image.size() / 512);
+					for (int m = 0; m < st.a_ops; m++)
+					{
+						const uint16_t* src = &plan.wsplit[(size_t)(op0 + m) * 512];
+						if (fold && WnFoldDead(m))
+						{
+							if (std::any_of(src, src + 512, [](uint16_t v) { return v != 0; })) throw std::runtime_error("internal: a folded layer's unused operand is not empty");
+							continue;
+						}
+						if (fold && first + WnFoldSlot(m) != (int)(image.size() / 512)) throw std::runtime_error("internal: folded operand out of place");
+						image.insert(image.end(), src, src + 512);
+					}
+					st.a_off = first * 64;
+					st.a_ops = (int)(image.size() / 512) - first;
+					if (fold && st.a_ops != WN_FOLD_OPS) throw std::runtime_error("internal: folded block size");
+				}
+				plan.wsplit.swap(image);
 			}
 
 			static WnSplitStage EmptySplit(int type)
@@ -576,6 +603,7 @@
 						prevHeadB = bh;
 					}
 				}
+				if (compactFold) CompactFoldedBlocks();
 				for (const WnSplitStage& st : plan.sstages) plan.maxSplitOps = std::max(plan.maxSplitOps, st.a_ops);
 				FinishRange();
 				plan.splitFastT = 2;
@@ -829,10 +857,11 @@
 		};
 	}
 
-	WaveNetPlan BuildWaveNetPlan(const WaveNetDesc& desc, bool splitStateFormat)
+	WaveNetPlan BuildWaveNetPlan(const WaveNetDesc& desc, bool splitStateFormat, bool compactFold)
 	{
 		Builder b(desc, 1, splitStateFormat);
 		b.foldOk = true;
+		b.compactFold = compactFold;
 		b.Build();
 		return std::move(b.plan);
 	}
diff --git a/neuralaudio_amd/csrc/wavenet_plan.h b/neuralaudio_amd/csrc/wavenet_plan.h
--- a/neuralaudio_amd/csrc/wavenet_plan.h
+++ b/neuralaudio_amd/csrc/wavenet_plan.h
@@ -52,7 +52,7 @@
 		std::vector<WnArrayCfg> arrays;
 	};
 
-	WaveNetPlan BuildWaveNetPlan(const WaveNetDesc& desc, bool splitStateFormat = false);
+	WaveNetPlan BuildWaveNetPlan(const WaveNetDesc& desc, bool splitStateFormat = false, bool compactFold = true);
 	void CheckWaveNetRunnable(const WaveNetDesc& desc);
 	int WaveNetPackFactor(const WaveNetDesc& desc);
 	bool WaveNetWantsPadding(const WaveNetDesc& desc);
diff --git a/neuralaudio_amd/csrc/wavenet_spec_impl.h b/neuralaudio_amd/csrc/wavenet_spec_impl.h
--- a/neuralaudio_amd/csrc/wavenet_spec_impl.h
+++ b/neuralaudio_amd/csrc/wavenet_spec_impl.h
@@ -77,6 +77,7 @@
 		{
 			static constexpr int SKEW = NA_SPK_SKEW;
 			static constexpr bool FOLD = true;
+			static constexpr int CHUNK = 9;
 			static constexpr int NA = 2;
 			static constexpr int CH[2] = { 16, 8 };
 			static constexpr int NLA[2] = { 10, 10 };
@@ -171,13 +172,15 @@
 					if (StageOfLayer(L) == s) return L;
 				return -1;
 			}
+			static constexpr bool FoldStage(int s) { return LayerOfStage(s) >= 0 && Fold(LayerOfStage(s)); }
+			static constexpr int OpSlot(int s, int m) { return FoldStage(s) ? WnFoldSlot(m) : m; }
 			static constexpr int StageOps(int s)
 			{
 				if (s == 0) return 1;
 				if (s == NSTAGES - 1) return 2 * HEADK + 1;
 				for (int a = 1; a < NA; a++)
 					if (s == LinkStage(a)) return 4 * LinkNC(a) + 1;
-				return 2 * KS(LayerOfStage(s)) + 4;
+				return FoldStage(s) ? WN_FOLD_OPS : 2 * KS(LayerOfStage(s)) + 4;
 			}
 			static constexpr int AOff(int s) { int o = 0; for (int i = 0; i < s; i++) o += StageOps(i) * 64; return o; }
 			static constexpr int WsplitQuads = AOff(NSTAGES);
@@ -205,11 +208,12 @@
 			static constexpr int MaxGP() { int m = 0; for (int a = 0; a < NA; a++) m = GPof(a) > m ? GPof(a) : m; return m; }
 		};
 
-		template <class A_, int NF_, int SPB_, bool PK_, bool COH_ = false, bool NT_ = false>
+		template <class A_, int NF_, int SPB_, bool PK_, bool COH_ = false, bool NT_ = false, bool QUAD_ = false>
 		struct Cfg
 		{
 			static constexpr bool COH = COH_;
 			static constexpr bool NT = NT_;
+			static constexpr bool QUAD = QUAD_;
 			typedef A_ A;
 			typedef Tab<A_> TB;
 			static constexpr int NF = NF_, T = A_::T, FW = 16 * T, WPS = NF_ / FW, SPB = SPB_ * T / 2, NTHREADS = 64 * WPS * SPB;
@@ -230,10 +234,11 @@
 			static constexpr int IDOP_OFF = WBUF_OFF + NWB * 2 * WBUF_ONE;
 			static constexpr int DUMP_OFF = IDOP_OFF + 1024;
 			static constexpr int FLAG_OFF = DUMP_OFF + 1024;
-			static constexpr int BCAST_OFF = FLAG_OFF + 16 * SPB;
+			static constexpr int BCAST_OFF = FLAG_OFF + (A_::LEAKY ? 16 * SPB : 0);
 			static constexpr int LDS_BYTES = BCAST_OFF + (COH_ ? 64 : 0);
 			static_assert(LDS_BYTES <= 80 * 1024, "two workgroups per CU");
 		};
+		static_assert(Cfg<ArchStd, 128, 1, false>::LDS_BYTES <= 40 * 1024, "four one-stream workgroups per CU");
 
 		template <int GP, int T>
 		struct Geo
@@ -628,8 +633,8 @@
 			constexpr int imgRead = s & 1, imgWrite = (s + 1) & 1, LN = SG::LN;
 			constexpr bool LASTLAYER = TB::LastOfArr(L) && TB::ArrOf(L) == TB::NA - 1;
 			constexpr int NEXTMINSHIFT = SG::NEXT ? TB::Dil(LN) : (1 << 20);
-			constexpr bool OWN = 2 * (K - 1) >= CB && 2 * (K - 1) < CE;
-			constexpr bool TAIL = 2 * K >= CB && 2 * K < CE;
+			constexpr bool OWN = SG::FOLD || (2 * (K - 1) >= CB && 2 * (K - 1) < CE);
+			constexpr bool TAIL = SG::FOLD || (2 * K >= CB && 2 * K < CE);
 			constexpr int LATER = ((OWN && SG::NEXT) ? HistLoadsOf<C, LN>() : 0) + ((TAIL && SG::NEXT && !LASTLAYER) ? StoresOf<C, LN>() : 0);
 			typedef typename NextChunk<C, s, c>::St NextStager;
 			if constexpr (c == 0)
@@ -643,7 +648,7 @@
 #pragma unroll
 				for (int i = 0; i < S; i++) ax[i] = AuxRead<C, GP>(ln, i);
 			}
-			constexpr int KLO = CB / 2, KHI = (CE / 2 < K - 1) ? CE / 2 : K - 1;
+			constexpr int KLO = CB / 2, KHI = (SG::FOLD || CE / 2 >= K - 1) ? K - 1 : CE / 2;
 			constexpr int NX = (KHI > C::HPF) ? KHI - (KLO > C::HPF ? KLO : C::HPF) : 0;
 			u32x4 hx[NX > 0 ? NX : 1][S];
 #pragma unroll
@@ -659,7 +664,7 @@
 #pragma unroll
 			for (int k = KLO; k < KHI; k++)
 			{
-				const u32x4 ah = WOp<C>(cx, s, c, 2 * k), al = SG::FOLD ? ah : WOp<C>(cx, s, c, 2 * k + 1);
+				const u32x4 ah = WOp<C>(cx, s, c, TB::OpSlot(s, 2 * k)), al = SG::FOLD ? ah : WOp<C>(cx, s, c, 2 * k + 1);
 #pragma unroll
 				for (int i = 0; i < S; i++)
 				{
@@ -672,14 +677,14 @@
 			}
 			if constexpr (SG::FOLD)
 			{
-				const u32x4 al01 = WOp<C>(cx, s, c, 1);
+				const u32x4 al01 = WOp<C>(cx, s, c, TB::OpSlot(s, 1));
 #pragma unroll
 				for (int i = 0; i < S; i++) acc[i] = Mfma(al01, u32x4{ th[0][i].x, th[0][i].y, th[1][i].x, th[1][i].y }, acc[i]);
 			}
 			if constexpr (OWN)
 			{
 				if constexpr (SG::NEXT) HistPrefetch<C, LN, WR>(cx, ln.ring, ln.fl, st);
-				const u32x4 ah = WOp<C>(cx, s, c, 2 * K - 2), al = WOp<C>(cx, s, c, 2 * K - 1);
+				const u32x4 ah = WOp<C>(cx, s, c, TB::OpSlot(s, 2 * K - 2)), al = WOp<C>(cx, s, c, TB::OpSlot(s, 2 * K - 1));
 #pragma unroll
 				for (int i = 0; i < S; i++)
 				{
@@ -702,11 +707,11 @@
 				for (int i = 0; i < S; i++)
 				{
 					if constexpr (C::A::LEAKY) z[i] = f32x4{ LeakyReLU(acc[i].x), LeakyReLU(acc[i].y), LeakyReLU(acc[i].z), LeakyReLU(acc[i].w) };
-					else z[i] = ActivateTanh<(NA_PK_TANH != 0) && (C::NTHREADS < 512)>(acc[i]);
+					else z[i] = ActivateTanh<(NA_PK_TANH != 0) && (C::NTHREADS < 512) && !C::QUAD>(acc[i]);
 				}
 				SPK_STAMP(s, 2);
 				const u32x4 idop = LdsRead16((unsigned)C::IDOP_OFF + (unsigned)cx.lane * 16u);
-				const u32x4 w1h = WOp<C>(cx, s, c, 2 * K + 1), w1l = WOp<C>(cx, s, c, 2 * K + 2), b1a = SG::FOLD ? w1l : WOp<C>(cx, s, c, 2 * K + 3);
+				const u32x4 w1h = WOp<C>(cx, s, c, TB::OpSlot(s, 2 * K + 1)), w1l = WOp<C>(cx, s, c, TB::OpSlot(s, 2 * K + 2)), b1a = SG::FOLD ? w1l : WOp<C>(cx, s, c, 2 * K + 3);
 #pragma unroll
 				for (int i = 0; i < S; i++)
 				{
@@ -1116,19 +1121,24 @@
 #ifndef NA_SPK_OCC
 #define NA_SPK_OCC(nf, spb) (((nf) * (spb) / 64) < 1 ? 1 : ((nf) * (spb) / 64))
 #endif
-		template <class F, int NF, int SPB>
-		constexpr int OccOf() { return F::A0::T == 1 ? (NA_SPK_OCC(NF, SPB) / 2 < 1 ? 1 : NA_SPK_OCC(NF, SPB) / 2) : NA_SPK_OCC(NF, SPB); }
-		template <class F, int NF, int SPB, bool PK, bool NT = false>
-		__global__ void __launch_bounds__(64 * (NF / (16 * F::A0::T)) * (SPB * F::A0::T / 2)) __attribute__((amdgpu_waves_per_eu(OccOf<F, NF, SPB>()))) WaveNetSpecKernel(const LaunchArgs args,
+		template <class F, int NF, int SPB, bool QUAD = false>
+		constexpr int OccOf()
+		{
+			if (QUAD) return 4;
+			return F::A0::T == 1 ? (NA_SPK_OCC(NF, SPB) / 2 < 1 ? 1 : NA_SPK_OCC(NF, SPB) / 2) : NA_SPK_OCC(NF, SPB);
+		}
+		template <class F, int NF, int SPB, bool PK, bool NT = false, bool QUAD = false>
+		__global__ void __launch_bounds__(64 * (NF / (16 * F::A0::T)) * (SPB * F::A0::T / 2)) __attribute__((amdgpu_waves_per_eu(OccOf<F, NF, SPB, QUAD>()))) WaveNetSpecKernel(const LaunchArgs args,
 			const float* __restrict__ in, float* __restrict__ out, long inStride, long outStride
 #ifdef NA_SP_TRACE
 			, long long* __restrict__ trace, int traceBlock
 #endif
 			)
 		{
-			typedef Cfg<typename F::A0, NF, SPB, PK, false, NT> C;
-			typedef Cfg<typename F::A1, NF, SPB, PK, false, NT> C1;
+			typedef Cfg<typename F::A0, NF, SPB, PK, false, NT, QUAD> C;
+			typedef Cfg<typename F::A1, NF, SPB, PK, false, NT, QUAD> C1;
 			static_assert(C::NTHREADS == C1::NTHREADS, "members of a family launch the same workgroup");
+			static_assert(!QUAD || 4 * (C::LDS_BYTES > C1::LDS_BYTES ? C::LDS_BYTES : C1::LDS_BYTES) <= 160 * 1024, "four workgroups per CU");
 			extern __shared__ __attribute__((aligned(16))) char dynSmem[];
 			asm volatile("" : : "s"((unsigned)(size_t)(LdsPtr)dynSmem));
 
@@ -1404,7 +1414,7 @@
 			return hipGetLastError();
 		}
 
-		template <class F, int NF, int SPB, bool PK, bool NT = false>
+		template <class F, int NF, int SPB, bool PK, bool NT = false, bool QUAD = false>
 		static hipError_t Launch(const WnFrameGroup* groups, int numGroups, const float* in, float* out, long inStride, long outStride, hipStream_t stream)
 		{
 			typedef Cfg<typename F::A0, NF, SPB, PK> C;
@@ -1417,10 +1427,10 @@
 			if (LDS_BYTES > 64 * 1024)
 			{
 				static PerDeviceOnce attr;
-				const hipError_t e = attr.Run([] { return hipFuncSetAttribute(reinterpret_cast<const void*>(WaveNetSpecKernel<F, NF, SPB, PK, NT>), hipFuncAttributeMaxDynamicSharedMemorySize, LDS_BYTES); });
+				const hipError_t e = attr.Run([] { return hipFuncSetAttribute(reinterpret_cast<const void*>(WaveNetSpecKernel<F, NF, SPB, PK, NT, QUAD>), hipFuncAttributeMaxDynamicSharedMemorySize, LDS_BYTES); });
 				if (e != hipSuccess) return e;
 			}
-			hipLaunchKernelGGL((WaveNetSpecKernel<F, NF, SPB, PK, NT>), dim3((unsigned)blocks), dim3(C::NTHREADS), LDS_BYTES, stream, args, in, out, inStride, outStride
+			hipLaunchKernelGGL((WaveNetSpecKernel<F, NF, SPB, PK, NT, QUAD>), dim3((unsigned)blocks), dim3(C::NTHREADS), LDS_BYTES, stream, args, in, out, inStride, outStride
 #ifdef NA_SP_TRACE
 				, GetWaveNetTraceBuffer(), Tuning::Get().traceBlock
 #endif
diff --git a/neuralaudio_amd/csrc/wavenet_spec_kernels.hip b/neuralaudio_amd/csrc/wavenet_spec_kernels.hip
--- a/neuralaudio_amd/csrc/wavenet_spec_kernels.hip
+++ b/neuralaudio_amd/csrc/wavenet_spec_kernels.hip
@@ -18,6 +18,15 @@
 		if (spk::Matches<spk::ArchA2Full>(stages, nstages, stateF4, wsplitQuads)) return WN_SPEC_A2FULL;
 		if (spk::Matches<spk::ArchA2Lite>(stages, nstages, stateF4, wsplitQuads)) return WN_SPEC_A2LITE;
 		return WN_SPEC_NONE;
+	}
+
+	void WaveNetSpecStdTables(int out[4])
+	{
+		typedef spk::Tab<spk::ArchStd> TB;
+		out[0] = TB::NSTAGES;
+		out[1] = TB::WsplitQuads;
+		out[2] = TB::StageOps(TB::StageOfLayer(0));
+		out[3] = spk::Cfg<spk::ArchStd, 128, 1, false>::LDS_BYTES;
 	}
 
 	hipError_t LaunchWaveNetSpecTable(const WnFrameGroup* groups, int numGroups, const float* in, float* out, long inStride, long outStride, int n,
@@ -93,10 +102,13 @@
 		const bool beyondCache = (sharing & WN_SHARING_BEYOND_CACHE) != 0;
 		sharing &= ~WN_SHARING_BEYOND_CACHE;
 		const int spb = spbEnv > 0 ? spbEnv : (halfGroups * std::max(sharing, 1) > residentHalf ? 2 : 1);
+		const bool quad = fam == 0 && arch == WN_SPEC_STD && n == 128 && !packed && !beyondCache && Tuning::Get().spQuad > 0;
 #ifdef NA_SP_QUICK
+		(void)quad;
 		if (arch != WN_SPEC_STD || packed) return hipErrorNotSupported;
 		return spk::LaunchNF<spk::FamStd, false>(groups, numGroups, in, out, inStride, outStride, n, spb, stream);
 #else
+		if (quad) return spk::Launch<spk::FamStd, 128, 1, false, false, true>(groups, numGroups, in, out, inStride, outStride, stream);
 		if (fam == 0) return packed ? hipErrorNotSupported : spk::LaunchNF<spk::FamStd, false>(groups, numGroups, in, out, inStride, outStride, n, spb, stream, beyondCache);
 		if (fam == 2) return packed ? hipErrorNotSupported : spk::LaunchSpecA2(groups, numGroups, in, out, inStride, outStride, n, spb, stream, beyondCache);
 		if (!packed && lite16) return hipErrorNotSupported;
diff --git a/neuralaudio_amd/csrc/wavenet_split_kernels.hip b/neuralaudio_amd/csrc/wavenet_split_kernels.hip
--- a/neuralaudio_amd/csrc/wavenet_split_kernels.hip
+++ b/neuralaudio_amd/csrc/wavenet_split_kernels.hip
@@ -247,13 +247,15 @@
 #pragma unroll
 				for (int i = 0; i < S; i++) acc[i] = f32x4{ 0.0f, 0.0f, 0.0f, 0.0f };
 				const bool fold = GP >= 2 && (sd.flags & WN_FLAG_FOLD) != 0;
+				auto wop = [&](int m) { return WOP(fold ? WnFoldSlot(m) : m); };
+				auto wopUnfolded = [&](int m) { return WOP(fold ? 0 : m); };
 				u32x2 th[2][S];
 #pragma unroll
 				for (int k = 0; k < HPF; k++)
 				{
 					if (!GEN || k < K - 1)
 					{
-						const u32x4 ah = wl[WOP(2 * k)], al = wl[WOP(2 * k + 1)];
+						const u32x4 ah = wl[wop(2 * k)], al = wl[wopUnfolded(2 * k + 1)];
 						const int shift = d * (K - 1 - k);
 						const int lo = cx.F0 - shift, hi = cx.F0 + 16 * P * S - 1 - shift;
 						if (hi < 0)
@@ -296,7 +298,7 @@
 				}
 				if (HPF >= 2 && fold)
 				{
-					const u32x4 al01 = wl[WOP(1)];
+					const u32x4 al01 = wl[wop(1)];
 #pragma unroll
 					for (int i = 0; i < S; i++) acc[i] = Mfma(al01, u32x4{ th[0][i].x, th[0][i].y, th[1][i].x, th[1][i].y }, acc[i]);
 				}
@@ -314,7 +316,7 @@
 				if constexpr (GEN)
 				for (int k = HPF; k < K - 1; k++)
 				{
-					const u32x4 ah = wl[WOP(2 * k)], al = wl[WOP(2 * k + 1)];
+					const u32x4 ah = wl[wop(2 * k)], al = wl[wopUnfolded(2 * k + 1)];
 					const int shift = d * (K - 1 - k);
 #pragma unroll
 					for (int i = 0; i < S; i++)
@@ -329,12 +331,12 @@
 				}
 				if (HPF < 2 && fold)
 				{
-					const u32x4 al01 = wl[WOP(1)];
+					const u32x4 al01 = wl[wop(1)];
 #pragma unroll
 					for (int i = 0; i < S; i++) acc[i] = Mfma(al01, u32x4{ th[0][i].x, th[0][i].y, th[1][i].x, th[1][i].y }, acc[i]);
 				}
 				{
-					const u32x4 ah = wl[WOP(2 * K - 2)], al = wl[WOP(2 * K - 1)], xa = wl[WOP(2 * K)];
+					const u32x4 ah = wl[wop(2 * K - 2)], al = wl[wop(2 * K - 1)], xa = wl[wopUnfolded(2 * K)];
 #pragma unroll
 					for (int i = 0; i < S; i++)
 					{
@@ -380,7 +382,7 @@
 				const bool pub = (sd.flags & WN_FLAG_PUBLISH) != 0;
 				const u32x4 idop = cx.idop[lane];
 				{
-					const u32x4 w1h = wl[WOP(2 * K + 1)], w1l = wl[WOP(2 * K + 2)], b1a = wl[WOP(2 * K + 3)];
+					const u32x4 w1h = wl[wop(2 * K + 1)], w1l = wl[wop(2 * K + 2)], b1a = wl[wopUnfolded(2 * K + 3)];
 #pragma unroll
 					for (int i = 0; i < S; i++)
 					{
```

New measurement: 3862, median of 3. 1.04x the previous value.
